# kolinko/effort

Hardware: AMD Instinct MI355X
Metric: effective GB/s + tokens/s vs effort %, Mistral-7B FFN 4096x11008 fp16 (higher is better)
Workload: dtype f16

## Files before the change

effort_amd/_lib.py:

```python
from __future__ import annotations

import ctypes as C
import os
import subprocess

_HERE = os.path.dirname(os.path.abspath(__file__))
LAB_LIB_PATH = os.path.join(_HERE, "libeffort_hip_lab.so")
LIB_PATH = (LAB_LIB_PATH if os.environ.get("EFFORT_HIP_LIB") == "lab" else os.environ.get("EFFORT_HIP_LIB")) or os.path.join(_HERE, "libeffort_hip.so")

ERRORS = {
    -1: "EFFORT_ERR_ARG", -2: "EFFORT_ERR_SHAPE", -3: "EFFORT_ERR_EFFORT", -4: "EFFORT_ERR_HIP",
    -5: "EFFORT_ERR_KIND", -6: "EFFORT_ERR_CONVERT", -7: "EFFORT_ERR_BLAS", -8: "EFFORT_ERR_COMM",
}


class EffortError(RuntimeError):
    def __init__(self, code: int, where: str, detail: str = ""):
        self.code = code
        super().__init__(f"{where}: {ERRORS.get(code, code)} {detail}".strip())


def build(verbose: bool = False) -> str:
    cmd = ["make", "-C", os.path.join(_HERE, "csrc"), "-j8", "all"]
    res = subprocess.run(cmd, capture_output=not verbose, text=True)
    if res.returncode != 0:
        raise RuntimeError("building libeffort_hip.so failed:\n" + (res.stdout or "") + (res.stderr or ""))
    return LIB_PATH


_P = C.c_void_p
_SIGS = {
    "effort_create": (_P, [C.c_int, _P]),
    "effort_destroy": (None, [_P]),
    "effort_set_stream": (C.c_int, [_P, _P]),
    "effort_sync": (C.c_int, [_P]),
    "effort_set_overlap": (C.c_int, [_P, C.c_int]),
    "effort_set_row_reuse": (C.c_int, [_P, C.c_int]),
    "effort_join": (C.c_int, [_P]),
    "effort_last_error": (C.c_char_p, [_P]),
    "effort_version": (C.c_char_p, []),
    "effort_weights_fp16": (_P, [_P, _P, _P, _P, C.c_int, C.c_int, C.c_int, C.c_int]),
    "effort_weights_fp16_pitched": (_P, [_P, _P, C.c_int, _P, _P, C.c_int, C.c_int, C.c_int, C.c_int]),
    "effort_aligned_row_pitch": (C.c_int, [C.c_int]),
    "effort_weights_q4": (_P, [_P, _P, _P, _P, _P, C.c_int64, C.c_int, C.c_int, C.c_int]),
    "effort_weights_free": (None, [_P]),
    "effort_weights_refresh": (C.c_int, [_P]),
    "effort_weights_align_rows": (C.c_int, [_P]),
    "effort_weights_row_pitch": (C.c_int, [_P]),
    "effort_weights_get_bound": (C.c_int, [_P, C.POINTER(C.c_float)]),
    "effort_weights_set_bound": (C.c_int, [_P, C.POINTER(C.c_float)]),
    "effort_weights_column_shard": (_P, [_P, C.c_int, C.c_int]),
    "effort_comm_unique_id": (C.c_int, [_P]),
    "effort_comm_create": (C.c_int, [_P, C.c_int, C.c_int, _P]),
    "effort_comm_destroy": (C.c_int, [_P]),
    "effort_comm_rank": (C.c_int, [_P]),
    "effort_comm_world": (C.c_int, [_P]),
    "effort_allgather_outputs": (C.c_int, [_P, _P, _P, C.c_int]),
    "effort_bucketmul": (C.c_int, [_P, _P, _P, _P, _P, C.c_double]),
    "effort_bucketmul_q4": (C.c_int, [_P, _P, _P, _P, _P, C.c_double]),
    "effort_bucketmul_group": (C.c_int, [_P, C.c_int, _P, _P, _P, _P, _P]),
    "effort_bucketmul_q4_group": (C.c_int, [_P, C.c_int, _P, _P, _P, _P, _P]),
    "effort_bucketmul_group_fused": (C.c_int, [_P, C.c_int, _P, _P, _P, _P, _P, _P, _P, _P]),
    "effort_bucketmul_q4_group_fused": (C.c_int, [_P, C.c_int, _P, _P, _P, _P, _P, _P, _P, _P]),
    "effort_group_dispatch_count": (C.c_int, [_P, C.c_int, C.POINTER(C.c_uint32)]),
    "effort_group_cutoff": (C.c_int, [_P, C.c_int, C.POINTER(C.c_float)]),
    "effort_debug_occupancy": (C.c_int, [_P, C.c_int, C.c_int, C.c_int, C.c_int]),
    "effort_set_persistent": (C.c_int, [_P, C.c_int]),
    "effort_debug_hook_lane": (C.c_int, [_P, C.c_int]),
    "effort_add_rmsnorm_mul": (C.c_int, [_P, _P, _P, _P, _P, C.c_int]),
    "effort_rope_kv": (C.c_int, [_P, _P, _P, _P, _P, _P, _P, _P, C.c_int, C.c_int, C.c_int, C.c_int, C.c_float]),
    "effort_attention": (C.c_int, [_P, _P, _P, _P, _P, _P, C.c_int, C.c_int, C.c_int]),
    "effort_rope_attention": (C.c_int, [_P, _P, _P, _P, _P, _P, _P, _P, C.c_int, C.c_int, C.c_int, C.c_int, C.c_float]),
    "effort_silu_mul": (C.c_int, [_P, _P, _P, _P, C.c_int]),
    "effort_fetch_row": (C.c_int, [_P, _P, _P, _P, C.c_int]),
    "effort_argmax": (C.c_int, [_P, _P, C.c_int, _P, _P, _P, C.c_int]),
    "effort_decode_status": (C.c_int, [_P, C.POINTER(C.c_int)]),
    "effort_sample": (C.c_int, [_P, _P, C.c_int, _P, _P, _P, _P, C.c_int, _P, _P]),
    "effort_topk": (C.c_int, [_P, _P, C.c_int, C.c_int, _P, _P]),
    "effort_sample_bits": (C.c_uint32, [C.c_uint32, C.c_uint32, C.c_uint32, C.c_uint32]),
    "effort_convert_status": (C.c_int, [_P, C.POINTER(C.c_int)]),
    "effort_q4_outlier_count": (C.c_int64, [C.c_int, C.c_int, C.c_double]),
    "effort_convert_q4": (C.c_int, [_P, _P, C.c_int, C.c_int, C.c_double, _P, _P, _P, _P]),
    "effort_top2_softmax": (C.c_int, [_P, _P, C.c_int, _P, _P]),
    "effort_mix2": (C.c_int, [_P, _P, _P, _P, _P, C.c_int]),
    "effort_moe_route": (C.c_int, [_P, _P, _P, _P, C.c_int, C.c_int, _P, _P, _P]),
    "effort_mix2_add": (C.c_int, [_P, _P, _P, _P, _P, C.c_int]),
    "effort_dense_gemv": (C.c_int, [_P, _P, _P, _P, C.c_int, C.c_int]),
    "effort_dense_gemv_expert": (C.c_int, [_P, _P, _P, _P, _P, C.c_int, C.c_int, C.c_int]),
    "effort_dense_gemm_rows": (C.c_int, [_P, _P, _P, _P, C.c_int, C.c_int, C.c_int]),
    "effort_dense_gemm_rows_routed": (C.c_int, [_P, _P, C.c_int, _P, _P, C.c_int, _P, C.c_int, C.c_int, C.c_int]),
    "effort_weights_bucket_dense_ok": (C.c_int, [_P, C.POINTER(C.c_int)]),
    "effort_bucket_gemm_rows": (C.c_int, [_P, _P, C.c_int, _P, _P, C.c_int]),
    "effort_bucket_gemm_rows_routed": (C.c_int, [_P, _P, _P, _P, C.c_int, _P, C.c_int]),
    "effort_moe_route_rows": (C.c_int, [_P, _P, _P, _P, C.c_int, C.c_int, _P, _P, _P, C.c_int]),
    "effort_mix2_add_rows": (C.c_int, [_P, _P, _P, _P, C.c_int, C.c_int]),
    "effort_fetch_rows": (C.c_int, [_P, _P, _P, _P, C.c_int, C.c_int]),
    "effort_add_rmsnorm_mul_rows": (C.c_int, [_P, _P, _P, _P, _P, C.c_int, C.c_int]),
    "effort_rope_kv_rows": (C.c_int, [_P, _P, _P, _P, _P, _P, _P, C.c_int, C.c_int, C.c_int, C.c_int, C.c_int, C.c_int, C.c_float]),
    "effort_attention_rows": (C.c_int, [_P, _P, _P, _P, C.c_int, C.c_int, _P, C.c_int, C.c_int, C.c_int]),
    "effort_attention_block": (C.c_int, [_P, _P, _P, _P, C.c_int, C.c_int, _P, C.c_int, C.c_int, C.c_int]),
    "effort_set_dense_backend": (C.c_int, [_P, C.c_int]),
    "effort_last_dispatch_count": (C.c_int, [_P, C.POINTER(C.c_uint32)]),
    "effort_last_cutoff": (C.c_int, [_P, C.POINTER(C.c_float)]),
    "effort_calc_dispatch": (C.c_int, [_P, _P, _P, _P, C.c_double, _P, _P]),
    "effort_convert_fp16": (C.c_int, [_P, _P, C.c_int, C.c_int, _P, _P, _P]),
    "effort_convert_fp16_pitched": (C.c_int, [_P, _P, C.c_int, C.c_int, _P, C.c_int, _P, _P]),
    "effort_cosine": (C.c_int, [_P, _P, _P, C.c_int, C.POINTER(C.c_float)]),
    "effort_set_split_cutoff": (C.c_int, [_P, C.c_int]),
    "effort_set_tuning": (C.c_int, [_P, C.c_int, C.c_int, C.c_int]),
    "effort_is_lab_build": (C.c_int, []),
    "effort_enable_kernel_timing": (C.c_int, [_P, C.c_int]),
    "effort_debug_stamps": (C.c_int, [_P, C.POINTER(C.c_ulonglong)]),
    "effort_debug_slice_counts": (C.c_int, [_P, C.c_int, C.POINTER(C.c_uint32), C.c_int]),
    "effort_debug_plan": (C.c_int, [C.c_int, C.c_int, C.c_int, C.c_int, _P, _P, _P, _P, _P, _P, C.c_int, C.c_int, C.c_int, C.c_int, _P, _P, _P, _P, _P, _P, _P, _P, _P]),
    "effort_debug_check_bundle": (C.c_int, [C.c_int, C.c_int, C.c_int, C.c_int, C.c_int, C.c_int]),
    "effort_debug_variants": (C.c_int, [C.c_int, _P, C.c_int]),
    "effort_debug_last_variant": (C.c_int, [_P, C.c_int, _P]),
    "effort_debug_lanes": (C.c_int, [C.c_int, C.c_int, _P, C.c_int64, _P]),
    "effort_debug_trace": (C.c_int, [_P, C.POINTER(C.c_ulonglong), C.c_int]),
    "effort_kernel_clock": (C.c_int, [_P, C.POINTER(C.c_double), C.POINTER(C.c_int)]),
    "effort_kernel_timing": (C.c_int, [_P, C.POINTER(C.c_double), C.POINTER(C.c_double), C.POINTER(C.c_double), C.POINTER(C.c_int)]),
}

_lib = None


def lib() -> C.CDLL:
    global _lib
    if _lib is None:
        if not os.path.exists(LIB_PATH):
            raise RuntimeError(
                f"{LIB_PATH} is missing: the HIP extension has not been built "
                "(run `python -c 'import __graft_entry__ as g; g.build()'` or `make -C effort_amd/csrc`). "
                "effort_amd has no CPU fallback.")
        import torch
        l = C.CDLL(LIB_PATH)
        for name, (res, args) in _SIGS.items():
            if (name.startswith("effort_debug_") or name == "effort_is_lab_build") and os.environ.get("EFFORT_HIP_LIB") and not hasattr(l, name):
                continue
            fn = getattr(l, name)
            fn.restype = res
            fn.argtypes = args
        _lib = l
    return _lib


def exported_symbols() -> list[str]:
    return sorted(_SIGS)
```

effort_amd/csrc/glue.hip:

```cpp
#include <rocblas/rocblas.h>

#include "host.h"
#include "prefill.h"
#include "sample_device.h"

using namespace effort;

extern "C" int effort_set_dense_backend(effort_ctx* c, int rocblas) {
    if (!c) return EFFORT_ERR_ARG;
    c->denseRocblas = rocblas != 0;
    return EFFORT_OK;
}
void dense_release(effort_ctx* c) { if (c->blas) rocblas_destroy_handle(c->blas); c->blas = nullptr; }
void dense_set_stream(effort_ctx* c) { if (c->blas) rocblas_set_stream(c->blas, c->stream); }
extern "C" int effort_dense_gemv(effort_ctx* c, const void* W, const float* v, float* out, int inDim, int outDim) {
    if (!c || !W || !v || !out || inDim <= 0 || outDim <= 0) return fail(c, EFFORT_ERR_ARG, "dense_gemv: bad argument");
    JOIN_TRY(c);
    if (inDim % 16) return fail(c, EFFORT_ERR_SHAPE, "dense_gemv: inDim % 16 != 0 (helpers/mps.swift:18)");
    if (!c->denseRocblas && dense_gemv_supported((uint32_t)inDim, (uint32_t)outDim)) {
        HIP_TRY(c, launch_dense_gemv(static_cast<const uint16_t*>(W), v, out, (uint32_t)inDim, (uint32_t)outDim, c->stream));
        return EFFORT_OK;
    }
    if (!c->blas) {
        if (rocblas_create_handle(&c->blas) != rocblas_status_success) return fail(c, EFFORT_ERR_BLAS, "rocblas_create_handle");
        rocblas_set_stream(c->blas, c->stream);
        rocblas_set_pointer_mode(c->blas, rocblas_pointer_mode_host);
    }
    OK_TRY(c->d_vhalf.grow(c, (size_t)inDim, (size_t)inDim));
    HIP_TRY(c, launch_f32_to_f16(v, c->d_vhalf.buf, inDim, c->stream));
    const float alpha = 1.0f, beta = 0.0f;
    rocblas_status s = rocblas_hssgemv_strided_batched(c->blas, rocblas_operation_transpose, inDim, outDim, &alpha,
                                                       static_cast<const rocblas_half*>(W), inDim, 0,
                                                       reinterpret_cast<const rocblas_half*>(c->d_vhalf.buf), 1, 0, &beta, out, 1, 0, 1);
    if (s != rocblas_status_success) return fail(c, EFFORT_ERR_BLAS, "rocblas_hssgemv_strided_batched");
    return EFFORT_OK;
}
extern "C" int effort_dense_gemv_expert(effort_ctx* c, const void* W, const uint32_t* expNo, const float* v, float* out, int inDim, int outDim,
                                        int numExperts) {
    if (!c || !W || !expNo || !v || !out || inDim <= 0 || outDim <= 0 || numExperts <= 0) return fail(c, EFFORT_ERR_ARG, "dense_gemv_expert: bad argument");
    JOIN_TRY(c);
    if (!dense_gemv_supported((uint32_t)inDim, (uint32_t)outDim) || (size_t)numExperts * outDim * inDim * 2 > 0xFFFFFFFFull)
        return fail(c, EFFORT_ERR_SHAPE, "dense_gemv_expert: inDim % 16 != 0, inDim > 65536, or a stack of 4 GiB or more");
    return HIP_RC(c, launch_dense_gemv_expert(static_cast<const uint16_t*>(W), expNo, v, out, (uint32_t)inDim, (uint32_t)outDim, (uint32_t)numExperts, c->stream));
}

extern "C" int effort_convert_fp16_pitched(effort_ctx* c, const void* W, int outDim, int inDim, void* buckets, int rowPitchBytes, void* stats, void* probes) {
    if (!c || !W || !buckets || !stats || !probes) return fail(c, EFFORT_ERR_ARG, "convert_fp16: null argument");
    JOIN_TRY(c);
    if (outDim <= 0 || inDim < kProbes || !(outDim >= kProbes || kProbes % outDim == 0) || outDim > 16384 || inDim > 32000 ||
        outDim % 16 || (outDim / 16) % 4)
        return fail(c, EFFORT_ERR_CONVERT, "convert_fp16: bucketize preconditions violated");
    const int pitch = rowPitchBytes ? rowPitchBytes : outDim / 16 * 2;
    if (pitch < outDim / 16 * 2 || pitch % 8) return fail(c, EFFORT_ERR_CONVERT, "convert_fp16: row pitch must be a multiple of 8 bytes >= 2*cols");
    const size_t elems = (size_t)outDim * inDim;
    OK_TRY(c->d_convVals.grow(c, elems, elems));
    return HIP_RC(c, launch_convert_fp16(static_cast<const uint16_t*>(W), outDim, inDim, static_cast<uint16_t*>(buckets), (uint32_t)pitch / 2u,
                                   static_cast<uint16_t*>(stats), static_cast<uint16_t*>(probes), c->d_convVals.buf, c->d_status, c->stream));
}
extern "C" int effort_convert_fp16(effort_ctx* c, const void* W, int outDim, int inDim, void* buckets, void* stats, void* probes) {
    return effort_convert_fp16_pitched(c, W, outDim, inDim, buckets, 0, stats, probes);
}

extern "C" int64_t effort_q4_outlier_count(int inDim, int outDim, double perc) {
    if (inDim <= 0 || outDim <= 0 || !(perc >= 0.0 && perc <= 1.0)) return EFFORT_ERR_ARG;
    return (int64_t)((double)((int64_t)inDim * outDim) * perc);
}
extern "C" int effort_convert_q4(effort_ctx* c, const void* core2, int inDim, int outDim, double perc, void* buckets, void* stats, void* probes,
                                 void* outliers) {
    if (!c || !core2 || !buckets || !stats || !probes) return fail(c, EFFORT_ERR_ARG, "convert_q4: null argument");
    JOIN_TRY(c);
    if (inDim <= 0 || outDim <= 0 || outDim % 32 || (int64_t)inDim * outDim >= (1ll << 32) || !(perc >= 0.0 && perc <= 1.0))
        return fail(c, EFFORT_ERR_CONVERT, "convert_q4: outDim % 32 != 0 (q4_draft.py:299), or a matrix of 2^32 elements or more");
    const int64_t cnt = effort_q4_outlier_count(inDim, outDim, perc);
    if (cnt >= (1ll << 31)) return fail(c, EFFORT_ERR_CONVERT, "convert_q4: 2^31 outliers or more (the candidate sort counts in int)");
    if (cnt > 0 && !outliers) return fail(c, EFFORT_ERR_ARG, "convert_q4: outliers buffer missing");
    hipSetDevice(c->device);
    return HIP_RC(c, launch_convert_q4(static_cast<const uint16_t*>(core2), (uint32_t)inDim, (uint32_t)outDim, (uint32_t)cnt, static_cast<uint16_t*>(buckets),
                                 static_cast<float*>(stats), static_cast<uint16_t*>(probes), static_cast<float*>(outliers), c->env.numCU, c->stream));
}

extern "C" int effort_cosine(effort_ctx* c, const float* a, const float* b, int n, float* host_out) {
    if (!c || !a || !b || !host_out || n <= 0) return EFFORT_ERR_ARG;
    JOIN_TRY(c);
    HIP_TRY(c, launch_cosine(a, b, n, c->d_cos, c->stream));
    HIP_TRY(c, hipMemcpyAsync(host_out, c->d_cos, 4, hipMemcpyDeviceToHost, c->stream));
    return HIP_RC(c, hipStreamSynchronize(c->stream));
}

extern "C" int effort_add_rmsnorm_mul(effort_ctx* c, float* h, const float* delta, const void* w, float* out, int n) {
    if (!c || !h || !w || !out || n <= 0) return fail(c, EFFORT_ERR_ARG, "add_rmsnorm_mul: bad argument");
    JOIN_TRY(c);
    return HIP_RC(c, launch_add_rmsnorm_mul(h, delta, static_cast<const uint16_t*>(w), out, (uint32_t)n, c->stream));
}
extern "C" int effort_rope_kv(effort_ctx* c, const float* xq, const float* xk, const float* xv, float* qOut, float* kCache,
                              float* vCache, const uint32_t* pos, int numHeads, int numHeadsKV, int headDim, int maxTokens, float ropeBase) {
    if (!c || !xq || !xk || !xv || !qOut || !kCache || !vCache || !pos) return fail(c, EFFORT_ERR_ARG, "rope_kv: null argument");
    JOIN_TRY(c);
    if (numHeads <= 0 || numHeadsKV <= 0 || numHeads % numHeadsKV || headDim < 2 || headDim > 1024 || headDim % 2 || !(ropeBase > 1.0f) || maxTokens <= 0)
        return fail(c, EFFORT_ERR_SHAPE, "rope_kv: bad head geometry");
    return HIP_RC(c, launch_rope_kv(xq, xk, xv, qOut, kCache, vCache, pos, numHeads, numHeadsKV, headDim, ropeBase, (uint32_t)maxTokens, c->d_status + 1, c->stream));
}
extern "C" int effort_attention(effort_ctx* c, const float* q, const float* kCache, const float* vCache, const uint32_t* pos,
                                float* out, int numHeads, int headDim, int maxTokens) {
    if (!c || !q || !kCache || !vCache || !pos || !out) return fail(c, EFFORT_ERR_ARG, "attention: null argument");
    JOIN_TRY(c);
    if (numHeads <= 0 || maxTokens <= 0 || maxTokens > 8192 || (headDim != 64 && headDim != 128 && headDim != 256))
        return fail(c, EFFORT_ERR_SHAPE, "attention: headDim 64/128/256, maxTokens <= 8192");
    return HIP_RC(c, launch_attention(q, kCache, vCache, pos, out, numHeads, headDim, maxTokens, c->stream));
}
extern "C" int effort_rope_attention(effort_ctx* c, const float* xq, const float* xk, const float* xv, float* kCache, float* vCache,
                                     const uint32_t* pos, float* out, int numHeads, int numHeadsKV, int headDim, int maxTokens, float ropeBase) {
    if (!c || !xq || !xk || !xv || !kCache || !vCache || !pos || !out) return fail(c, EFFORT_ERR_ARG, "rope_attention: null argument");
    JOIN_TRY(c);
    if (numHeads <= 0 || numHeadsKV <= 0 || numHeads % numHeadsKV || maxTokens <= 0 || maxTokens > 8192 || !(ropeBase > 1.0f) ||
        (headDim != 64 && headDim != 128 && headDim != 256))
        return fail(c, EFFORT_ERR_SHAPE, "rope_attention: headDim 64/128/256, maxTokens <= 8192");
    return HIP_RC(c, launch_rope_attention(xq, xk, xv, kCache, vCache, pos, out, numHeads, numHeadsKV, headDim, maxTokens, ropeBase, c->d_status + 1, c->stream));
}
extern "C" int effort_silu_mul(effort_ctx* c, const float* x1, const float* x3, float* out, int n) {
    if (!c || !x1 || !x3 || !out || n <= 0) return fail(c, EFFORT_ERR_ARG, "silu_mul: bad argument");
    JOIN_TRY(c);
    return HIP_RC(c, launch_silu_mul(x1, x3, out, (uint32_t)n, c->stream));
}
extern "C" int effort_fetch_row(effort_ctx* c, const void* emb, const uint32_t* id, float* out, int n) {
    if (!c || !emb || !id || !out || n <= 0) return fail(c, EFFORT_ERR_ARG, "fetch_row: bad argument");
    JOIN_TRY(c);
    return HIP_RC(c, launch_fetch_row(static_cast<const uint16_t*>(emb), id, out, (uint32_t)n, c->stream));
}
static_assert(EFFORT_PREFILL_MAX_ROWS == 64, "prefill.hip: kPrefillMaxRows, four token tiles of 16");
static bool prefill_rows_ok(int rows) { return rows >= 1 && rows <= EFFORT_PREFILL_MAX_ROWS; }
extern "C" int effort_dense_gemm_rows(effort_ctx* c, const void* W, const float* x, float* out, int inDim, int outDim, int rows) {
    if (inDim <= 0 || outDim <= 0 || !prefill_rows_ok(rows)) return fail(c, EFFORT_ERR_ARG, "dense_gemm_rows: inDim, outDim >= 1, 1 <= rows <= 64");
    if (!dense_gemm_rows_supported((uint32_t)inDim, (uint32_t)outDim))
        return fail(c, EFFORT_ERR_SHAPE, "dense_gemm_rows: inDim % 32 == 0, inDim <= 65536, outDim <= 2^24, W below 4 GiB");
    if (!c || !W || !x || !out) return fail(c, EFFORT_ERR_ARG, "dense_gemm_rows: null argument");
    JOIN_TRY(c);
    OK_TRY(c->d_xhRows.grow(c, (size_t)rows * inDim, (size_t)EFFORT_PREFILL_MAX_ROWS * inDim));
    OK_TRY(c->d_gemmPart.grow(c, dense_gemm_rows_partial_floats((uint32_t)inDim, (uint32_t)outDim, (uint32_t)rows),
                              dense_gemm_rows_partial_floats((uint32_t)inDim, (uint32_t)outDim, EFFORT_PREFILL_MAX_ROWS)));
    return HIP_RC(c, launch_dense_gemm_rows(static_cast<const uint16_t*>(W), x, c->d_xhRows.buf, c->d_gemmPart.buf, out, (uint32_t)inDim, (uint32_t)outDim,
                                      (uint32_t)rows, c->stream));
}
extern "C" int effort_dense_gemm_rows_routed(effort_ctx* c, const void* W, int numExperts, const uint32_t* idx2, const float* x, int xPerSlot, float* out,
                                             int inDim, int outDim, int rows) {
    if (inDim <= 0 || outDim <= 0 || numExperts <= 0 || !prefill_rows_ok(rows) || (xPerSlot != 0 && xPerSlot != 1))
        return fail(c, EFFORT_ERR_ARG, "dense_gemm_rows_routed: inDim, outDim, numExperts >= 1, 1 <= rows <= 64, xPerSlot 0 / 1");
    if (!dense_gemm_rows_supported((uint32_t)inDim, (uint32_t)outDim) || numExperts > 64)
        return fail(c, EFFORT_ERR_SHAPE, "dense_gemm_rows_routed: inDim % 32 == 0, inDim <= 65536, outDim <= 2^24, one expert below 4 GiB, numExperts <= 64");
    if (!c || !W || !idx2 || !x || !out) return fail(c, EFFORT_ERR_ARG, "dense_gemm_rows_routed: null argument");
    JOIN_TRY(c);
    const size_t xRows = (size_t)(xPerSlot ? 2 : 1) * rows;
    OK_TRY(c->d_xhRouted.grow(c, xRows * inDim, (size_t)2 * EFFORT_PREFILL_MAX_ROWS * inDim));
    OK_TRY(c->d_routedPart.grow(c, dense_gemm_rows_routed_partial_floats((uint32_t)inDim, (uint32_t)outDim, (uint32_t)rows),
                                dense_gemm_rows_routed_partial_floats((uint32_t)inDim, (uint32_t)outDim, EFFORT_PREFILL_MAX_ROWS)));
    OK_TRY(c->d_routedGroups.grow(c, dense_gemm_rows_routed_group_words(), dense_gemm_rows_routed_group_words()));
    return HIP_RC(c, launch_dense_gemm_rows_routed(static_cast<const uint16_t*>(W), (uint32_t)numExperts, idx2, x, (uint32_t)xPerSlot, c->d_xhRouted.buf,
                                             c->d_routedPart.buf, c->d_routedGroups.buf, out, (uint32_t)inDim, (uint32_t)outDim, (uint32_t)rows, c->stream));
}
static int bucket_handle_shape(const effort_w* w, const char* name) {
    char what[128];
    if (w->fmt != kFp16) { snprintf(what, sizeof(what), "%s: an FP16 bundle (Q4 buckets hold no whole matrix)", name); return fail(w->ctx, EFFORT_ERR_KIND, what); }
    if (w->rowsPerIn != 16u || w->view || w->inDim % 32u || !bucket_gemm_rows_supported(w->inDim, w->outDim)) {
        snprintf(what, sizeof(what), "%s: percentLoad 16, a full handle (no column shard), inDim %% 32 == 0", name);
        return fail(w->ctx, EFFORT_ERR_SHAPE, what);
    }
    return EFFORT_OK;
}
static int bucket_dense_state(const effort_w* w, int* ok) {
    effort_ctx* c = w->ctx;
    if (w->bucketDense < 0) {
        int bad = 0;
        hipSetDevice(c->device);
        JOIN_TRY(c);
        HIP_TRY(c, hipMemsetAsync(c->d_status + 2, 0, 4, c->stream));
        HIP_TRY(c, launch_bucket_dense_check(w->buckets, w->rowPitch, w->cols, w->inDim, w->numExperts, c->d_status + 2, c->stream));
        HIP_TRY(c, hipMemcpyAsync(&bad, c->d_status + 2, 4, hipMemcpyDeviceToHost, c->stream));
        HIP_TRY(c, hipStreamSynchronize(c->stream));
        w->bucketDense = bad ? 0 : 1;
    }
    *ok = w->bucketDense;
    return EFFORT_OK;
}
extern "C" int effort_weights_bucket_dense_ok(effort_w* w, int* host_out) {
    if (!w || !w->ctx || w->dead || !host_out) return EFFORT_ERR_ARG;
    OK_TRY(bucket_handle_shape(w, "weights_bucket_dense_ok"));
    return bucket_dense_state(w, host_out);
}
static int bucket_refuse_collisions(effort_ctx* c, const effort_w* w, const char* name) {
    int ok = 0;
    OK_TRY(bucket_dense_state(w, &ok));
    if (ok) return EFFORT_OK;
    char what[160];
    snprintf(what, sizeof(what), "%s: the bundle is not un-bucketable (two entries of one bucket name the same output: effort_convert_status reported drops)", name);
    return fail(c, EFFORT_ERR_CONVERT, what);
}
extern "C" int effort_bucket_gemm_rows(effort_ctx* c, const effort_w* w, int expert, const float* x, float* out, int rows) {
    if (!w || w->dead) return fail(c, EFFORT_ERR_ARG, "bucket_gemm_rows: null handle");
    if (!prefill_rows_ok(rows) || expert < 0 || (uint32_t)expert >= w->numExperts) return fail(c, EFFORT_ERR_ARG, "bucket_gemm_rows: 1 <= rows <= 64, 0 <= expert < numExperts");
    OK_TRY(bucket_handle_shape(w, "bucket_gemm_rows"));
    if (!c || c != w->ctx || !x || !out) return fail(c, EFFORT_ERR_ARG, "bucket_gemm_rows: null argument (or a handle of another context)");
    JOIN_TRY(c);
    OK_TRY(bucket_refuse_collisions(c, w, "bucket_gemm_rows"));
    OK_TRY(c->d_xhRows.grow(c, (size_t)rows * w->inDim, (size_t)EFFORT_PREFILL_MAX_ROWS * w->inDim));
    OK_TRY(c->d_gemmPart.grow(c, dense_gemm_rows_partial_floats(w->inDim, w->outDim, (uint32_t)rows),
                              dense_gemm_rows_partial_floats(w->inDim, w->outDim, EFFORT_PREFILL_MAX_ROWS)));
    const uint16_t* B = reinterpret_cast<const uint16_t*>(reinterpret_cast<const unsigned char*>(w->buckets) + (size_t)expert * 16u * w->inDim * w->rowPitch);
    return HIP_RC(c, launch_bucket_gemm_rows(B, w->rowPitch, x, c->d_xhRows.buf, c->d_gemmPart.buf, out, w->inDim, w->outDim, (uint32_t)rows, c->stream));
}
extern "C" int effort_bucket_gemm_rows_routed(effort_ctx* c, const effort_w* w, const uint32_t* idx2, const float* x, int xPerSlot, float* out, int rows) {
    if (!w || w->dead) return fail(c, EFFORT_ERR_ARG, "bucket_gemm_rows_routed: null handle");
    if (!prefill_rows_ok(rows) || (xPerSlot != 0 && xPerSlot != 1)) return fail(c, EFFORT_ERR_ARG, "bucket_gemm_rows_routed: 1 <= rows <= 64, xPerSlot 0 / 1");
    OK_TRY(bucket_handle_shape(w, "bucket_gemm_rows_routed"));
    if (w->numExperts > 64u) return fail(c, EFFORT_ERR_SHAPE, "bucket_gemm_rows_routed: numExperts <= 64");
    if (!c || c != w->ctx || !idx2 || !x || !out) return fail(c, EFFORT_ERR_ARG, "bucket_gemm_rows_routed: null argument (or a handle of another context)");
    JOIN_TRY(c);
    OK_TRY(bucket_refuse_collisions(c, w, "bucket_gemm_rows_routed"));
    const size_t xRows = (size_t)(xPerSlot ? 2 : 1) * rows;
    OK_TRY(c->d_xhRouted.grow(c, xRows * w->inDim, (size_t)2 * EFFORT_PREFILL_MAX_ROWS * w->inDim));
    OK_TRY(c->d_routedPart.grow(c, dense_gemm_rows_routed_partial_floats(w->inDim, w->outDim, (uint32_t)rows),
                                dense_gemm_rows_routed_partial_floats(w->inDim, w->outDim, EFFORT_PREFILL_MAX_ROWS)));
    OK_TRY(c->d_routedGroups.grow(c, dense_gemm_rows_routed_group_words(), dense_gemm_rows_routed_group_words()));
    return HIP_RC(c, launch_bucket_gemm_rows_routed(w->buckets, w->rowPitch, w->numExperts, idx2, x, (uint32_t)xPerSlot, c->d_xhRouted.buf, c->d_routedPart.buf,
                                              c->d_routedGroups.buf, out, w->inDim, w->outDim, (uint32_t)rows, c->stream));
}
extern "C" int effort_moe_route_rows(effort_ctx* c, const float* h, const void* normW, const void* gateW, int n, int numExperts, float* gateOut,
                                     uint32_t* idx2, float* val2, int rows) {
    if (n <= 0 || numExperts <= 0 || !prefill_rows_ok(rows)) return fail(c, EFFORT_ERR_ARG, "moe_route_rows: n, numExperts >= 1, 1 <= rows <= 64");
    if (!moe_route_supported((uint32_t)n, (uint32_t)numExperts))
        return fail(c, EFFORT_ERR_SHAPE, "moe_route_rows: n % 16 == 0, 16 <= n <= 16384, 1 <= numExperts <= 64");
    if (!c || !h || !normW || !gateW || !idx2 || !val2) return fail(c, EFFORT_ERR_ARG, "moe_route_rows: null argument");
    JOIN_TRY(c);
    return HIP_RC(c, launch_moe_route_rows(h, static_cast<const uint16_t*>(normW), static_cast<const uint16_t*>(gateW), (uint32_t)n, (uint32_t)numExperts, gateOut,
                                     idx2, val2, (uint32_t)rows, c->stream));
}
extern "C" int effort_mix2_add_rows(effort_ctx* c, float* h, const float* f, const float* val2, int n, int rows) {
    if (n <= 0 || !prefill_rows_ok(rows)) return fail(c, EFFORT_ERR_ARG, "mix2_add_rows: n >= 1, 1 <= rows <= 64");
    if (!c || !h || !f || !val2) return fail(c, EFFORT_ERR_ARG, "mix2_add_rows: null argument");
    JOIN_TRY(c);
    return HIP_RC(c, launch_mix2_add_rows(h, f, val2, (uint32_t)n, (uint32_t)rows, c->stream));
}
extern "C" int effort_fetch_rows(effort_ctx* c, const void* emb, const uint32_t* ids, float* out, int n, int rows) {
    if (n <= 0 || !prefill_rows_ok(rows)) return fail(c, EFFORT_ERR_ARG, "fetch_rows: n >= 1, 1 <= rows <= 64");
    if (!c || !emb || !ids || !out) return fail(c, EFFORT_ERR_ARG, "fetch_rows: null argument");
    JOIN_TRY(c);
    return HIP_RC(c, launch_fetch_rows(static_cast<const uint16_t*>(emb), ids, out, (uint32_t)n, (uint32_t)rows, c->stream));
}
extern "C" int effort_add_rmsnorm_mul_rows(effort_ctx* c, float* h, const float* delta, const void* w, float* out, int n, int rows) {
    if (n <= 0 || !prefill_rows_ok(rows)) return fail(c, EFFORT_ERR_ARG, "add_rmsnorm_mul_rows: n >= 1, 1 <= rows <= 64");
    if (!c || !h || !w || !out) return fail(c, EFFORT_ERR_ARG, "add_rmsnorm_mul_rows: null argument");
    JOIN_TRY(c);
    return HIP_RC(c, launch_add_rmsnorm_mul_rows(h, delta, static_cast<const uint16_t*>(w), out, (uint32_t)n, (uint32_t)rows, c->stream));
}
static bool prefill_range_ok(int pos0, int rows, int maxTokens) {
    return prefill_rows_ok(rows) && pos0 >= 0 && maxTokens > 0 && pos0 <= maxTokens - rows;
}
extern "C" int effort_rope_kv_rows(effort_ctx* c, const float* xq, const float* xk, const float* xv, float* qOut, float* kCache, float* vCache,
                                   int pos0, int rows, int numHeads, int numHeadsKV, int headDim, int maxTokens, float ropeBase) {
    if (!prefill_range_ok(pos0, rows, maxTokens)) return fail(c, EFFORT_ERR_ARG, "rope_kv_rows: 1 <= rows <= 64, 0 <= pos0, pos0 + rows <= maxTokens");
    if (numHeads <= 0 || numHeadsKV <= 0 || numHeads % numHeadsKV || headDim < 2 || headDim > 1024 || headDim % 2 || !(ropeBase > 1.0f))
        return fail(c, EFFORT_ERR_SHAPE, "rope_kv_rows: bad head geometry");
    if (!c || !xq || !xk || !xv || !qOut || !kCache || !vCache) return fail(c, EFFORT_ERR_ARG, "rope_kv_rows: null argument");
    JOIN_TRY(c);
    return HIP_RC(c, launch_rope_kv_rows(xq, xk, xv, qOut, kCache, vCache, (uint32_t)pos0, (uint32_t)rows, numHeads, numHeadsKV, headDim, ropeBase, c->stream));
}
static int prefill_attention(effort_ctx* c, const char* name, decltype(&launch_attention_rows) launch, const float* q, const float* kCache,
                             const float* vCache, int pos0, int rows, float* out, int numHeads, int headDim, int maxTokens) {
    char what[96];
    auto refuse = [&](int code, const char* why) { snprintf(what, sizeof(what), "%s: %s", name, why); return fail(c, code, what); };
    if (!prefill_range_ok(pos0, rows, maxTokens)) return refuse(EFFORT_ERR_ARG, "1 <= rows <= 64, 0 <= pos0, pos0 + rows <= maxTokens");
    if (numHeads <= 0 || maxTokens > 8192 || (headDim != 64 && headDim != 128 && headDim != 256))
        return refuse(EFFORT_ERR_SHAPE, "headDim 64/128/256, maxTokens <= 8192");
    if (!c || !q || !kCache || !vCache || !out) return refuse(EFFORT_ERR_ARG, "null argument");
    JOIN_TRY(c);
    return hip_rc(c, name, launch(q, kCache, vCache, (uint32_t)pos0, (uint32_t)rows, out, numHeads, headDim, c->stream));
}
extern "C" int effort_attention_rows(effort_ctx* c, const float* q, const float* kCache, const float* vCache, int pos0, int rows, float* out,
                                     int numHeads, int headDim, int maxTokens) {
    return prefill_attention(c, "attention_rows", launch_attention_rows, q, kCache, vCache, pos0, rows, out, numHeads, headDim, maxTokens);
}
extern "C" int effort_attention_block(effort_ctx* c, const float* q, const float* kCache, const float* vCache, int pos0, int rows, float* out,
                                      int numHeads, int headDim, int maxTokens) {
    return prefill_attention(c, "attention_block", launch_attention_block, q, kCache, vCache, pos0, rows, out, numHeads, headDim, maxTokens);
}
extern "C" int effort_top2_softmax(effort_ctx* c, const float* gate, int n, uint32_t* idx2, float* val2) {
    if (!c || !gate || !idx2 || !val2 || n < 1) return fail(c, EFFORT_ERR_ARG, "top2_softmax: bad argument");
    JOIN_TRY(c);
    return HIP_RC(c, launch_top2_softmax(gate, (uint32_t)n, idx2, val2, c->stream));
}
extern "C" int effort_mix2(effort_ctx* c, const float* f0, const float* f1, const float* val2, float* out, int n) {
    if (!c || !f0 || !f1 || !val2 || !out || n <= 0) return fail(c, EFFORT_ERR_ARG, "mix2: bad argument");
    JOIN_TRY(c);
    return HIP_RC(c, launch_mix2(f0, f1, val2, out, (uint32_t)n, c->stream));
}
extern "C" int effort_moe_route(effort_ctx* c, const float* h, const void* normW, const void* gateW, int n, int numExperts, float* gateOut,
                                uint32_t* idx2, float* val2) {
    if (!c || !h || !normW || !gateW || !idx2 || !val2) return fail(c, EFFORT_ERR_ARG, "moe_route: null argument");
    JOIN_TRY(c);
    if (n <= 0 || numExperts <= 0 || !moe_route_supported((uint32_t)n, (uint32_t)numExperts))
        return fail(c, EFFORT_ERR_SHAPE, "moe_route: n % 16 == 0, 16 <= n <= 16384, 1 <= numExperts <= 64");
    return HIP_RC(c, launch_moe_route(h, static_cast<const uint16_t*>(normW), static_cast<const uint16_t*>(gateW), (uint32_t)n, (uint32_t)numExperts, gateOut,
                                idx2, val2, c->stream));
}
extern "C" int effort_mix2_add(effort_ctx* c, float* h, const float* f0, const float* f1, const float* val2, int n) {
    if (!c || !h || !f0 || !f1 || !val2 || n <= 0) return fail(c, EFFORT_ERR_ARG, "mix2_add: bad argument");
    JOIN_TRY(c);
    return HIP_RC(c, launch_mix2_add(h, f0, f1, val2, (uint32_t)n, c->stream));
}
extern "C" int effort_argmax(effort_ctx* c, const float* logits, int n, uint32_t* idOut, uint32_t* pos, uint32_t* history, int historyLen) {
    if (!c || !logits || !idOut || !pos || n <= 0 || (history && historyLen <= 0)) return fail(c, EFFORT_ERR_ARG, "argmax: bad argument");
    JOIN_TRY(c);
    return HIP_RC(c, launch_argmax(logits, (uint32_t)n, idOut, pos, history, (uint32_t)(history ? historyLen : 0), c->d_status + 1, c->stream));
}
extern "C" int effort_sample(effort_ctx* c, const float* logits, int n, const effort_sample_params* params, uint32_t* idOut, uint32_t* pos,
                             uint32_t* history, int historyLen, uint32_t* topkIdx, float* topkVal) {
    if (!c || !logits || !params || !idOut || !pos || n <= 0 || (history && historyLen <= 0)) return fail(c, EFFORT_ERR_ARG, "sample: bad argument");
    JOIN_TRY(c);
    return HIP_RC(c, launch_sample(logits, (uint32_t)n, params, idOut, pos, history, (uint32_t)(history ? historyLen : 0), c->d_status + 1, topkIdx, topkVal,
                             c->stream));
}
extern "C" int effort_topk(effort_ctx* c, const float* logits, int n, int k, uint32_t* idx, float* val) {
    if (!c || !logits || !idx || !val || n <= 0 || k < 1 || k > EFFORT_SAMPLE_MAX_K) return fail(c, EFFORT_ERR_ARG, "topk: bad argument (1 <= k <= 64)");
    JOIN_TRY(c);
    return HIP_RC(c, launch_topk(logits, (uint32_t)n, (uint32_t)k, idx, val, c->stream));
}
extern "C" uint32_t effort_sample_bits(uint32_t seedLo, uint32_t seedHi, uint32_t stream, uint32_t pos) { return philox_x0(seedLo, seedHi, stream, pos); }

static int read_and_clear(effort_ctx* c, int* word, int* host_out) {
    if (!c || !host_out) return EFFORT_ERR_ARG;
    JOIN_TRY(c);
    HIP_TRY(c, hipMemcpyAsync(host_out, word, 4, hipMemcpyDeviceToHost, c->stream));
    HIP_TRY(c, hipMemsetAsync(word, 0, 4, c->stream));
    return HIP_RC(c, hipStreamSynchronize(c->stream));
}
extern "C" int effort_decode_status(effort_ctx* c, int* host_out) { return read_and_clear(c, c ? c->d_status + 1 : nullptr, host_out); }
extern "C" int effort_convert_status(effort_ctx* c, int* host_out) { return read_and_clear(c, c ? c->d_status : nullptr, host_out); }
```

effort_amd/csrc/host.h:

```cpp
#pragma once
#include <cstdio>
#include <cstring>
#include <new>

#include "../../include/effort_hip.h"
#include "../../include/effort_hip_debug.h"
#include "effort_internal.h"
#include "lanes.h"
#include "plan.h"

struct ncclComm;
struct _rocblas_handle;

struct Lane {
    hipStream_t own = nullptr;
    hipEvent_t done = nullptr;
    bool dirty = false;
    float* d_cutoff = nullptr;
    uint32_t* d_count = nullptr;
    float* d_slabs = nullptr;
    uint32_t* d_counters = nullptr;
    uint32_t* d_sliceCounts = nullptr;
    uint32_t* d_queue = nullptr;
    uint32_t lastCalls = 1, lastSliceOff[effort::kMaxGroup] = {0}, lastSlices[effort::kMaxGroup] = {0};
    uint32_t lastLaunches = 0;
    effort::LaunchedVariant lastVariant[effort::kMaxLaunches] = {};
};

template <typename T>
struct Scratch {
    T* buf = nullptr;
    size_t have = 0;
    int grow(effort_ctx* c, size_t need, size_t want);
    void release() { hipFree(buf); buf = nullptr; have = 0; }
};
#define EFFORT_CTX_SCRATCH(X)                                                                                                              \
    X(uint16_t, d_vhalf)                                                                         \
    X(uint16_t, d_xhRows)        \
    X(float, d_gemmPart)                                                           \
    X(uint16_t, d_xhRouted)      \
    X(float, d_routedPart) X(uint32_t, d_routedGroups)          \
    X(uint16_t, d_convVals)

struct effort_ctx {
    static constexpr uint32_t kMaxTiles = 1024, kMaxSlices = 4096;
    static constexpr size_t kSlabBytes = (size_t)64 << 20;
    int device = 0;
    hipStream_t stream = nullptr;
    effort::PlanEnv env = scratch_env();
    static effort::PlanEnv scratch_env() { effort::PlanEnv e; e.slabBytes = kSlabBytes; e.maxTiles = kMaxTiles; e.maxSlices = kMaxSlices; return e; }
    Lane lane[effort::kMaxLanes];
    effort::LaneBook book;
    int lastLane = 0;
    hipEvent_t forkEv = nullptr;
    uint32_t* d_blockScratch = nullptr;
#define EFFORT_X(T, name) Scratch<T> name;
    EFFORT_CTX_SCRATCH(EFFORT_X)
#undef EFFORT_X
    float* d_cos = nullptr;
    int* d_status = nullptr;
    unsigned long long* d_tstamp = nullptr;
    double wallClockKHz = 100000.0;
    _rocblas_handle* blas = nullptr;
    ncclComm* comm = nullptr;
    int commRank = 0, commWorld = 1;
    bool denseRocblas = false;
    bool rowReuse = false;
    bool timing = false;
    bool trace = false;
    static constexpr int kMaxSamples = 4096;
    hipEvent_t* ev = nullptr;
    int nSamples = 0;
    char err[256] = {0};
};

struct effort_w {
    effort_ctx* ctx = nullptr;
    effort::Format fmt = effort::kFp16;
    const uint16_t* buckets = nullptr;
    const uint16_t* bucketsSrc = nullptr;
    uint16_t* aligned = nullptr;
    uint32_t rowPitch = 0;
    uint32_t srcPitch = 0;
    const void* stats = nullptr;
    const uint16_t* probes = nullptr;
    uint32_t inDim = 0, outDim = 0, rowsPerIn = 0, numExperts = 1, cols = 0;
    bool view = false;
    effort_w* parent = nullptr;
    uint32_t viewTrim = 0;
    int views = 0;
    bool dead = false;
    float* rankBound = nullptr;
    uint16_t* means16 = nullptr;
    mutable int bucketDense = -1;
    uint64_t nOutliers = 0;
    uint32_t* olBlockPtr = nullptr;
    uint32_t* olEntry = nullptr;
    uint32_t* olMeta = nullptr;
};

static inline int fail(effort_ctx* c, int code, const char* what, hipError_t e = hipSuccess) {
    if (c) {
        if (e != hipSuccess) snprintf(c->err, sizeof(c->err), "%s: %s", what, hipGetErrorString(e));
        else snprintf(c->err, sizeof(c->err), "%s", what);
    }
    return code;
}
static inline int hip_rc(effort_ctx* c, const char* what, hipError_t e) { return e == hipSuccess ? EFFORT_OK : fail(c, EFFORT_ERR_HIP, what, e); }
#define HIP_RC(ctx, call) hip_rc((ctx), #call, (call))
#define OK_TRY(step) do { const int rc_ = (step); if (rc_ != EFFORT_OK) return rc_; } while (0)
#define HIP_TRY(ctx, call) OK_TRY(HIP_RC(ctx, call))
#define JOIN_TRY(ctx) OK_TRY(join_lanes(ctx))

template <typename T>
int Scratch<T>::grow(effort_ctx* c, size_t need, size_t want) {
    if (need <= have) return EFFORT_OK;
    HIP_TRY(c, hipStreamSynchronize(c->stream));
    release();
    HIP_TRY(c, hipMalloc(&buf, want * sizeof(T)));
    have = want;
    return EFFORT_OK;
}

int join_lanes(effort_ctx* c);
struct LaneChoice {
    bool laned = false;
    effort::LanePick pick;
    effort::LaunchRanges ranges;
    unsigned long long capNow = 0;
    bool forked = false;
};
int choose_lane(effort_ctx* c, LaneChoice& lc, int n, const effort_w* const* ws, const float* const* vs, const uint32_t* const* expNos,
                float* const* outs, const void* const* vAux, const float* const* resids);
int fork_lane(effort_ctx* c, LaneChoice& lc);
int check_shape(uint32_t inDim, uint32_t outDim);
int check_bundle(effort::Format fmt, int inDim, int outDim, int percentLoad, int numExperts, int rowPitchBytes, uint32_t* pitchOut);
void comm_release(effort_ctx* c);
void dense_release(effort_ctx* c);
void dense_set_stream(effort_ctx* c);
```

effort_amd/csrc/prefill.h:

```cpp
#pragma once
#include "effort_internal.h"

namespace effort {

constexpr int kPrefillMaxRows = 64;
constexpr uint32_t kPfStage = 256;
constexpr size_t kPfKeepBytes = 64u << 20;
constexpr uint32_t kPfMaxAssign = 2u * kPrefillMaxRows, kPfMaxExperts = 64;

typedef _Float16 pf_half8 __attribute__((ext_vector_type(8)));
typedef float pf_f32x4 __attribute__((ext_vector_type(4)));

struct PfSplit { uint32_t per, splits; };
PfSplit pf_split(uint32_t inDim, uint32_t outDim);

hipError_t launch_rows_to_f16(const float* x, uint16_t* xh, uint32_t n, hipStream_t st);
hipError_t launch_reduce_splits(const float* part, float* out, uint32_t n, uint32_t splits, hipStream_t st);
hipError_t launch_routed_prologue(const float* x, uint16_t* xh, uint32_t n, const uint32_t* idx2, uint32_t assigns, uint32_t numExperts, uint32_t* cnt,
                                  uint32_t* list, hipStream_t st);

bool bucket_gemm_rows_supported(uint32_t inDim, uint32_t outDim);
hipError_t launch_bucket_dense_check(const uint16_t* B, uint32_t pitch, uint32_t cols, uint32_t inDim, uint32_t numExperts, int* bad, hipStream_t st);
hipError_t launch_bucket_gemm_rows(const uint16_t* B, uint32_t pitch, const float* x, uint16_t* xh, float* part, float* out, uint32_t inDim,
                                   uint32_t outDim, uint32_t rows, hipStream_t st);
hipError_t launch_bucket_gemm_rows_routed(const uint16_t* B, uint32_t pitch, uint32_t numExperts, const uint32_t* idx2, const float* x, uint32_t xPerSlot,
                                          uint16_t* xh, float* part, uint32_t* groups, float* out, uint32_t inDim, uint32_t outDim, uint32_t rows,
                                          hipStream_t st);

}
```

effort_amd/csrc/prefill_buckets.hip:

```cpp
#include <type_traits>

#include "prefill.h"

namespace effort {

constexpr uint32_t kBkCols = 32;
constexpr uint32_t kBkRows = 16u * kBkCols;
constexpr uint32_t kBkWaves = 8, kBkThreads = 64u * kBkWaves;
constexpr uint32_t kBkTiles = kBkRows / 16u / kBkWaves;
constexpr uint32_t kBkK = 64;
constexpr uint32_t kBkPitch = kBkK * 2u + 16u;
constexpr uint32_t kBkTileBytes = kBkRows * kBkPitch;
constexpr uint32_t kBkLds = kBkTileBytes + 64u * kBkPitch;
static_assert(kPfStage % kBkK == 0 && kBkTileBytes % (16u * kBkThreads) == 0, "whole chunks per stage; the fill is whole 16-byte stores");

template <int NT, int AUX, int VEC, bool ROUTED>
__device__ __forceinline__ void bucket_rows_body(unsigned char* __restrict__ lds, const uint16_t* __restrict__ B, uint32_t pitch, uint32_t cols,
                                                 const uint16_t* __restrict__ xh, float* __restrict__ o, uint32_t inDim, uint32_t outDim, uint32_t live,
                                                 uint32_t xRows, uint32_t per, const uint32_t* col, uint32_t xShift) {
    constexpr uint32_t kPiecesPerRow = kBkCols * 2u / (4u * VEC);
    constexpr int kLoads = (int)(16u * kBkK * kPiecesPerRow / kBkThreads);
    constexpr uint32_t kXPieces = NT * 16u * (kBkK / 8u);
    constexpr int kXLoads = (int)((kXPieces + kBkThreads - 1u) / kBkThreads);
    unsigned char* const tile = lds;
    unsigned char* const xs = lds + kBkTileBytes;
    const uint32_t tid = threadIdx.x, lane = tid & 63u, wave = __builtin_amdgcn_readfirstlane(tid >> 6);
    const uint32_t g = lane >> 4, r16 = lane & 15u, c0 = blockIdx.x * kBkCols;
    const __amdgpu_buffer_rsrc_t rs = __builtin_amdgcn_make_buffer_rsrc(const_cast<uint16_t*>(B), 0, (int)((16u * inDim - 1u) * pitch + cols * 2u), 0x00020000);
    const __amdgpu_buffer_rsrc_t xr = __builtin_amdgcn_make_buffer_rsrc(const_cast<uint16_t*>(xh), 0, (int)(xRows * inDim * 2u), 0x00020000);
    const uint32_t chunks = (inDim + kPfStage - 1u) / kPfStage * (kPfStage / kBkK);
    const uint32_t q0 = blockIdx.y * per * (kPfStage / kBkK), q1 = min(q0 + per * (kPfStage / kBkK), chunks);

    constexpr int kDepth = VEC == 4 && !ROUTED ? 2 : 1;
    uint32_t heldA[kDepth][kLoads][VEC];
    uint4 heldX[kDepth][kXLoads];
    auto ask_a = [&](uint32_t q, uint32_t (&nextA)[kLoads][VEC]) {
#pragma unroll
        for (int i = 0; i < kLoads; i++) {
            const uint32_t idx = tid + (uint32_t)i * kBkThreads, brow = idx / kPiecesPerRow, p = idx % kPiecesPerRow;
            const uint32_t rank = brow / kBkK, j = q * kBkK + brow % kBkK, cFirst = c0 + p * 2u * VEC;
#pragma unroll
            for (int v = 0; v < VEC; v++) nextA[i][v] = 0u;
            if (j < inDim && cFirst + 2u * VEC <= cols) {
                const uint32_t off = (rank * inDim + j) * pitch + cFirst * 2u;
                if constexpr (VEC == 4) {
                    const auto w = __builtin_amdgcn_raw_buffer_load_b128(rs, off, 0, AUX);
                    nextA[i][0] = w[0]; nextA[i][1] = w[1]; nextA[i][2] = w[2]; nextA[i][3] = w[3];
                } else {
                    nextA[i][0] = __builtin_amdgcn_raw_buffer_load_b32(rs, off, 0, AUX);
                }
            }
        }
    };
    auto x_row = [&](uint32_t tok) -> uint32_t {
        if constexpr (ROUTED) return tok < live ? col[tok] >> xShift : 0u;
        else return min(tok, live - 1u);
    };
    auto ask_x = [&](uint32_t q, uint4 (&nextX)[kXLoads]) {
#pragma unroll
        for (int i = 0; i < kXLoads; i++) {
            const uint32_t idx = tid + (uint32_t)i * kBkThreads, tok = idx / (kBkK / 8u), e = q * kBkK + (idx % (kBkK / 8u)) * 8u;
            nextX[i] = make_uint4(0u, 0u, 0u, 0u);
            if (idx < kXPieces && tok < live && e < inDim) {
                const auto x = __builtin_amdgcn_raw_buffer_load_b128(xr, x_row(tok) * inDim * 2u + e * 2u, 0, 0);
                nextX[i] = make_uint4(x[0], x[1], x[2], x[3]);
            }
        }
    };
    auto scatter = [&](const uint32_t (&nextA)[kLoads][VEC], const uint4 (&nextX)[kXLoads]) {
#pragma unroll
        for (int i = 0; i < kLoads; i++) {
            const uint32_t idx = tid + (uint32_t)i * kBkThreads, brow = idx / kPiecesPerRow, p = idx % kPiecesPerRow;
            const uint32_t jj = brow % kBkK, cLocal = p * 2u * VEC;
#pragma unroll
            for (int v = 0; v < VEC; v++)
#pragma unroll
                for (int h = 0; h < 2; h++) {
                    const uint32_t w = (nextA[i][v] >> (16 * h)) & 0xFFFFu;
                    const uint32_t row = (cLocal + 2u * v + h) * 16u + (w & 15u);
                    if (w != 0u) *reinterpret_cast<uint16_t*>(tile + row * kBkPitch + jj * 2u) = (uint16_t)w;
                }
        }
#pragma unroll
        for (int i = 0; i < kXLoads; i++) {
            const uint32_t idx = tid + (uint32_t)i * kBkThreads;
            if (idx < kXPieces) *reinterpret_cast<uint4*>(xs + (idx / (kBkK / 8u)) * kBkPitch + (idx % (kBkK / 8u)) * 16u) = nextX[i];
        }
    };

    pf_f32x4 acc[kBkTiles][NT];
#pragma unroll
    for (int m = 0; m < (int)kBkTiles; m++)
#pragma unroll
        for (int t = 0; t < NT; t++) acc[m][t] = pf_f32x4{0.0f, 0.0f, 0.0f, 0.0f};
    auto chunk = [&](uint32_t q, auto slotTag) {
        constexpr int slot = decltype(slotTag)::value;
#pragma unroll
        for (int i = 0; i < (int)(kBkTileBytes / (16u * kBkThreads)); i++)
            *reinterpret_cast<uint4*>(tile + (tid + (uint32_t)i * kBkThreads) * 16u) = make_uint4(0u, 0u, 0u, 0u);
        __syncthreads();
        scatter(heldA[slot], heldX[slot]);
        __syncthreads();
        if (q + kDepth < q1) { ask_a(q + kDepth, heldA[slot]); ask_x(q + kDepth, heldX[slot]); }
        __builtin_amdgcn_sched_barrier(0);
#pragma unroll
        for (int u = 0; u < 2; u++) {
            pf_half8 bf[NT];
#pragma unroll
            for (int t = 0; t < NT; t++) bf[t] = *reinterpret_cast<const pf_half8*>(xs + (t * 16u + r16) * kBkPitch + (g * 2u + u) * 16u);
#pragma unroll
            for (int m = 0; m < (int)kBkTiles; m++) {
                const pf_half8 af = *reinterpret_cast<const pf_half8*>(tile + ((wave * kBkTiles + m) * 16u + r16) * kBkPitch + (g * 2u + u) * 16u);
#pragma unroll
                for (int t = 0; t < NT; t++) acc[m][t] = __builtin_amdgcn_mfma_f32_16x16x32_f16(af, bf[t], acc[m][t], 0, 0, 0);
            }
        }
        __builtin_amdgcn_sched_barrier(0);
        __syncthreads();
    };
    ask_a(q0, heldA[0]);
    ask_x(q0, heldX[0]);
    if constexpr (kDepth == 2) {
        if (q0 + 1u < q1) { ask_a(q0 + 1u, heldA[1]); ask_x(q0 + 1u, heldX[1]); }
        for (uint32_t q = q0; q < q1; q += 2u) {
            chunk(q, std::integral_constant<int, 0>{});
            if (q + 1u < q1) chunk(q + 1u, std::integral_constant<int, 1>{});
        }
    } else {
        for (uint32_t q = q0; q < q1; q++) chunk(q, std::integral_constant<int, 0>{});
    }
#pragma unroll
    for (int t = 0; t < NT; t++) {
        const uint32_t tok = t * 16u + r16;
        uint32_t orow = tok;
        if constexpr (ROUTED) orow = tok < live ? col[tok] : 0u;
#pragma unroll
        for (int m = 0; m < (int)kBkTiles; m++)
#pragma unroll
            for (int i = 0; i < 4; i++) {
                const uint32_t row = c0 * 16u + (wave * kBkTiles + m) * 16u + g * 4u + i;
                if (tok < live && row < outDim) o[(size_t)orow * outDim + row] = acc[m][t][i];
            }
    }
}

template <int NT, int AUX, int VEC>
__global__ __launch_bounds__(kBkThreads) void bucket_gemm_rows_kernel(const uint16_t* __restrict__ B, uint32_t pitch, uint32_t cols,
                                                                      const uint16_t* __restrict__ xh, float* __restrict__ dst, uint32_t inDim,
                                                                      uint32_t outDim, uint32_t rows, uint32_t per) {
    extern __shared__ __attribute__((aligned(16))) unsigned char bk_lds[];
    bucket_rows_body<NT, AUX, VEC, false>(bk_lds, B, pitch, cols, xh, dst + (size_t)blockIdx.y * rows * outDim, inDim, outDim, rows, rows, per, nullptr, 0u);
}

template <int AUX, int VEC>
__global__ __launch_bounds__(kBkThreads) void bucket_gemm_rows_routed_kernel(const uint16_t* __restrict__ B, uint32_t pitch, uint32_t cols,
                                                                             const uint16_t* __restrict__ xh, float* __restrict__ dst,
                                                                             const uint32_t* __restrict__ cnt, const uint32_t* __restrict__ list,
                                                                             uint32_t inDim, uint32_t outDim, uint32_t assigns, uint32_t xRows,
                                                                             uint32_t xShift, uint32_t per) {
    extern __shared__ __attribute__((aligned(16))) unsigned char bk_lds[];
    __shared__ uint32_t col[64];
    const uint32_t e = blockIdx.z, n = __builtin_amdgcn_readfirstlane(min(cnt[e], kPfMaxAssign));
    if (n == 0u) return;
    const uint16_t* Be = reinterpret_cast<const uint16_t*>(reinterpret_cast<const unsigned char*>(B) + (size_t)e * 16u * inDim * pitch);
    float* o = dst + (size_t)blockIdx.y * assigns * outDim;
    for (uint32_t a0 = 0; a0 < n; a0 += 64u) {
        const uint32_t live = min(n - a0, 64u);
        if (threadIdx.x < live) col[threadIdx.x] = min(list[e * kPfMaxAssign + a0 + threadIdx.x], assigns - 1u);
        __syncthreads();
        switch ((live + 15u) / 16u) {
            case 1: bucket_rows_body<1, AUX, VEC, true>(bk_lds, Be, pitch, cols, xh, o, inDim, outDim, live, xRows, per, col, xShift); break;
            case 2: bucket_rows_body<2, AUX, VEC, true>(bk_lds, Be, pitch, cols, xh, o, inDim, outDim, live, xRows, per, col, xShift); break;
            case 3: bucket_rows_body<3, AUX, VEC, true>(bk_lds, Be, pitch, cols, xh, o, inDim, outDim, live, xRows, per, col, xShift); break;
            default: bucket_rows_body<4, AUX, VEC, true>(bk_lds, Be, pitch, cols, xh, o, inDim, outDim, live, xRows, per, col, xShift); break;
        }
        __syncthreads();
    }
}

__global__ __launch_bounds__(256) void bucket_dense_check_kernel(const uint16_t* __restrict__ B, uint32_t pitch, uint32_t cols, uint32_t inDim, int* bad) {
    const uint32_t cp = blockIdx.x * 256u + threadIdx.x, j = blockIdx.y, e = blockIdx.z;
    if (cp >= cols / 2u) return;
    const unsigned char* base = reinterpret_cast<const unsigned char*>(B) + ((size_t)e * 16u * inDim + j) * pitch + cp * 4u;
    uint32_t seen0 = 0u, seen1 = 0u, dup = 0u;
    for (uint32_t r = 0; r < 16u; r++) {
        const uint32_t w = *reinterpret_cast<const uint32_t*>(base + (size_t)r * inDim * pitch), w0 = w & 0xFFFFu, w1 = w >> 16;
        const uint32_t b0 = w0 ? 1u << (w0 & 15u) : 0u, b1 = w1 ? 1u << (w1 & 15u) : 0u;
        dup |= (seen0 & b0) | (seen1 & b1);
        seen0 |= b0; seen1 |= b1;
    }
    if (dup) atomicOr(bad, 1);
}

bool bucket_gemm_rows_supported(uint32_t inDim, uint32_t outDim) {
    return dense_gemm_rows_supported(inDim, outDim) && outDim % 32u == 0 && outDim <= 16384u;
}

hipError_t launch_bucket_dense_check(const uint16_t* B, uint32_t pitch, uint32_t cols, uint32_t inDim, uint32_t numExperts, int* bad, hipStream_t st) {
    hipLaunchKernelGGL(bucket_dense_check_kernel, dim3((cols / 2u + 255u) / 256u, inDim, numExperts), dim3(256), 0, st, B, pitch, cols, inDim, bad);
    return hipGetLastError();
}

static bool bucket_wide(const uint16_t* B, uint32_t pitch, uint32_t cols) {
    return pitch % 16u == 0 && reinterpret_cast<uintptr_t>(B) % 16u == 0 && cols % 8u == 0;
}

template <int NT, int AUX, int VEC>
static hipError_t launch_bucket_gemm_rows_t(const uint16_t* B, uint32_t pitch, uint32_t cols, const uint16_t* xh, float* dst, uint32_t inDim,
                                            uint32_t outDim, uint32_t rows, PfSplit sp, hipStream_t st) {
    const hipError_t e = allow_full_lds(reinterpret_cast<const void*>(&bucket_gemm_rows_kernel<NT, AUX, VEC>));
    if (e != hipSuccess) return e;
    hipLaunchKernelGGL((bucket_gemm_rows_kernel<NT, AUX, VEC>), dim3((cols + kBkCols - 1u) / kBkCols, sp.splits), dim3(kBkThreads), kBkLds, st,
                       B, pitch, cols, xh, dst, inDim, outDim, rows, sp.per);
    return hipGetLastError();
}
template <int NT>
static hipError_t launch_bucket_gemm_rows_nt(bool nt, bool wide, const uint16_t* B, uint32_t pitch, uint32_t cols, const uint16_t* xh, float* dst,
                                             uint32_t inDim, uint32_t outDim, uint32_t rows, PfSplit sp, hipStream_t st) {
    if (nt) return wide ? launch_bucket_gemm_rows_t<NT, 2, 4>(B, pitch, cols, xh, dst, inDim, outDim, rows, sp, st)
                        : launch_bucket_gemm_rows_t<NT, 2, 1>(B, pitch, cols, xh, dst, inDim, outDim, rows, sp, st);
    return wide ? launch_bucket_gemm_rows_t<NT, 0, 4>(B, pitch, cols, xh, dst, inDim, outDim, rows, sp, st)
                : launch_bucket_gemm_rows_t<NT, 0, 1>(B, pitch, cols, xh, dst, inDim, outDim, rows, sp, st);
}

hipError_t launch_bucket_gemm_rows(const uint16_t* B, uint32_t pitch, const float* x, uint16_t* xh, float* part, float* out, uint32_t inDim,
                                   uint32_t outDim, uint32_t rows, hipStream_t st) {
    if (rows < 1u || rows > (uint32_t)kPrefillMaxRows) return hipErrorInvalidValue;
    hipError_t e = launch_rows_to_f16(x, xh, rows * inDim, st);
    if (e != hipSuccess) return e;
    const PfSplit sp = pf_split(inDim, outDim);
    float* dst = sp.splits > 1u ? part : out;
    const uint32_t cols = outDim / 16u;
    const bool nt = (size_t)inDim * outDim * 2u > kPfKeepBytes, wide = bucket_wide(B, pitch, cols);
    switch ((rows + 15u) / 16u) {
        case 1: e = launch_bucket_gemm_rows_nt<1>(nt, wide, B, pitch, cols, xh, dst, inDim, outDim, rows, sp, st); break;
        case 2: e = launch_bucket_gemm_rows_nt<2>(nt, wide, B, pitch, cols, xh, dst, inDim, outDim, rows, sp, st); break;
        case 3: e = launch_bucket_gemm_rows_nt<3>(nt, wide, B, pitch, cols, xh, dst, inDim, outDim, rows, sp, st); break;
        default: e = launch_bucket_gemm_rows_nt<4>(nt, wide, B, pitch, cols, xh, dst, inDim, outDim, rows, sp, st); break;
    }
    if (e != hipSuccess || sp.splits == 1u) return e;
    return launch_reduce_splits(part, out, rows * outDim, sp.splits, st);
}

template <int AUX, int VEC>
static hipError_t launch_bucket_gemm_rows_routed_t(const uint16_t* B, uint32_t pitch, uint32_t cols, uint32_t numExperts, const uint16_t* xh, float* dst,
                                                   const uint32_t* cnt, const uint32_t* list, uint32_t inDim, uint32_t outDim, uint32_t assigns,
                                                   uint32_t xRows, uint32_t xShift, PfSplit sp, hipStream_t st) {
    const hipError_t e = allow_full_lds(reinterpret_cast<const void*>(&bucket_gemm_rows_routed_kernel<AUX, VEC>));
    if (e != hipSuccess) return e;
    hipLaunchKernelGGL((bucket_gemm_rows_routed_kernel<AUX, VEC>), dim3((cols + kBkCols - 1u) / kBkCols, sp.splits, numExperts), dim3(kBkThreads), kBkLds, st,
                       B, pitch, cols, xh, dst, cnt, list, inDim, outDim, assigns, xRows, xShift, sp.per);
    return hipGetLastError();
}

hipError_t launch_bucket_gemm_rows_routed(const uint16_t* B, uint32_t pitch, uint32_t numExperts, const uint32_t* idx2, const float* x, uint32_t xPerSlot,
                                          uint16_t* xh, float* part, uint32_t* groups, float* out, uint32_t inDim, uint32_t outDim, uint32_t rows,
                                          hipStream_t st) {
    if (rows < 1u || rows > (uint32_t)kPrefillMaxRows || numExperts < 1u || numExperts > kPfMaxExperts || xPerSlot > 1u) return hipErrorInvalidValue;
    const uint32_t assigns = 2u * rows, xRows = xPerSlot ? assigns : rows, cols = outDim / 16u;
    uint32_t* cnt = groups;
    uint32_t* list = groups + kPfMaxExperts;
    hipError_t e = launch_routed_prologue(x, xh, xRows * inDim, idx2, assigns, numExperts, cnt, list, st);
    if (e != hipSuccess) return e;
    const PfSplit sp = pf_split(inDim, outDim);
    float* dst = sp.splits > 1u ? part : out;
    const uint32_t xShift = xPerSlot ? 0u : 1u;
    const bool nt = (size_t)inDim * outDim * 2u > kPfKeepBytes;
    const bool wide = bucket_wide(B, pitch, cols);
    if (nt) e = wide ? launch_bucket_gemm_rows_routed_t<2, 4>(B, pitch, cols, numExperts, xh, dst, cnt, list, inDim, outDim, assigns, xRows, xShift, sp, st)
                     : launch_bucket_gemm_rows_routed_t<2, 1>(B, pitch, cols, numExperts, xh, dst, cnt, list, inDim, outDim, assigns, xRows, xShift, sp, st);
    else e = wide ? launch_bucket_gemm_rows_routed_t<0, 4>(B, pitch, cols, numExperts, xh, dst, cnt, list, inDim, outDim, assigns, xRows, xShift, sp, st)
                  : launch_bucket_gemm_rows_routed_t<0, 1>(B, pitch, cols, numExperts, xh, dst, cnt, list, inDim, outDim, assigns, xRows, xShift, sp, st);
    if (e != hipSuccess || sp.splits == 1u) return e;
    return launch_reduce_splits(part, out, assigns * outDim, sp.splits, st);
}

}
```

include/effort_hip_debug.h:

```cpp
#ifndef EFFORT_HIP_DEBUG_H
#define EFFORT_HIP_DEBUG_H

#include "effort_hip.h"

#ifdef __cplusplus
extern "C" {
#endif

EFFORT_API int effort_set_tuning(effort_ctx* ctx, int wavesPerGroup, int elemsPerLane, int rowSlices);
EFFORT_API int effort_set_split_cutoff(effort_ctx* ctx, int split);

EFFORT_API int effort_set_persistent(effort_ctx* ctx, int wgPerCU);

EFFORT_API int effort_debug_hook_lane(effort_ctx* ctx, int lane);

EFFORT_API int effort_is_lab_build(void);
EFFORT_API int effort_enable_kernel_timing(effort_ctx* ctx, int enable);
EFFORT_API int effort_kernel_clock(effort_ctx* ctx, double* mul_us_avg, int* n_launches);
EFFORT_API int effort_kernel_timing(effort_ctx* ctx, double* mul_us_avg, double* cutoff_us_avg,
                         double* integrate_us_avg, int* n_samples);
EFFORT_API int effort_debug_occupancy(effort_ctx* ctx, int q4, int waves, int elems, int ldsBytes);
EFFORT_API int effort_debug_stamps(effort_ctx* ctx, unsigned long long* host32);
EFFORT_API int effort_debug_slice_counts(effort_ctx* ctx, int idx, uint32_t* host, int maxSlices);
EFFORT_API int effort_debug_plan(int q4, int numCU, int lanes, int n, const int* inDim, const int* outDim, const int* percentLoad,
                      const int* prologue, const int* hasResid, const double* effort, int persistent, int tuneW, int tuneE, int tuneS,
                      int* we, int* slices, int* tiles, int* sliceRows, int* launchOf,
                      int* launchPersistent, int* launchCutJobs, int* launchCompact, int* launchStagger);
EFFORT_API int effort_debug_check_bundle(int q4, int inDim, int outDim, int percentLoad, int numExperts, int rowPitchBytes);
EFFORT_API int effort_debug_variants(int q4, int* rows, int maxRows);
EFFORT_API int effort_debug_last_variant(effort_ctx* ctx, int launch, int* out8);
#define EFFORT_LANES_LAUNCH 0
#define EFFORT_LANES_TIMED 1
#define EFFORT_LANES_JOIN 2
#define EFFORT_LANES_OUT_WORDS 18
EFFORT_API int effort_debug_lanes(int lanes, int nOps, const int64_t* ops, int64_t nWords, int64_t* out);
EFFORT_API int effort_debug_trace(effort_ctx* ctx, unsigned long long* host, int maxRecords);

#ifdef __cplusplus
}
#endif
#endif
```

Measured before the change: 22220.

## Retile bucket prefill GEMM with adaptive column groups and double-buffered LDS

Reworks the bucket GEMM-rows prefill kernel. Column-group width is now a template parameter (4–32 columns) picked by a cost model over CU count, with a debug override. Each WG runs 4 waves, double-buffers LDS for small groups, uses a deeper prefetch pipeline and load widths matched to the group, and swizzles the block index across 64-column lines. The fill path becomes branchless, with zero rows stored into a dummy slot, and non-temporal load hints are dropped. The aim is better occupancy and load/compute overlap for prefill, at the cost of more template variants and a heuristic that could pick a poor group size.

```diff
diff --git a/effort_amd/_lib.py b/effort_amd/_lib.py
--- a/effort_amd/_lib.py
+++ b/effort_amd/_lib.py
@@ -116,6 +116,8 @@
     "effort_debug_check_bundle": (C.c_int, [C.c_int, C.c_int, C.c_int, C.c_int, C.c_int, C.c_int]),
     "effort_debug_variants": (C.c_int, [C.c_int, _P, C.c_int]),
     "effort_debug_last_variant": (C.c_int, [_P, C.c_int, _P]),
+    "effort_debug_bucket_group": (C.c_int, [C.c_int, C.c_int, C.c_int]),
+    "effort_debug_set_bucket_group": (C.c_int, [_P, C.c_int]),
     "effort_debug_lanes": (C.c_int, [C.c_int, C.c_int, _P, C.c_int64, _P]),
     "effort_debug_trace": (C.c_int, [_P, C.POINTER(C.c_ulonglong), C.c_int]),
     "effort_kernel_clock": (C.c_int, [_P, C.POINTER(C.c_double), C.POINTER(C.c_int)]),
diff --git a/effort_amd/csrc/glue.hip b/effort_amd/csrc/glue.hip
--- a/effort_amd/csrc/glue.hip
+++ b/effort_amd/csrc/glue.hip
@@ -205,7 +205,8 @@
     OK_TRY(c->d_gemmPart.grow(c, dense_gemm_rows_partial_floats(w->inDim, w->outDim, (uint32_t)rows),
                               dense_gemm_rows_partial_floats(w->inDim, w->outDim, EFFORT_PREFILL_MAX_ROWS)));
     const uint16_t* B = reinterpret_cast<const uint16_t*>(reinterpret_cast<const unsigned char*>(w->buckets) + (size_t)expert * 16u * w->inDim * w->rowPitch);
-    return HIP_RC(c, launch_bucket_gemm_rows(B, w->rowPitch, x, c->d_xhRows.buf, c->d_gemmPart.buf, out, w->inDim, w->outDim, (uint32_t)rows, c->stream));
+    return HIP_RC(c, launch_bucket_gemm_rows(B, w->rowPitch, x, c->d_xhRows.buf, c->d_gemmPart.buf, out, w->inDim, w->outDim, (uint32_t)rows,
+                                             (uint32_t)c->env.numCU, c->bucketGroup, c->stream));
 }
 extern "C" int effort_bucket_gemm_rows_routed(effort_ctx* c, const effort_w* w, const uint32_t* idx2, const float* x, int xPerSlot, float* out, int rows) {
     if (!w || w->dead) return fail(c, EFFORT_ERR_ARG, "bucket_gemm_rows_routed: null handle");
@@ -221,7 +222,18 @@
                                 dense_gemm_rows_routed_partial_floats(w->inDim, w->outDim, EFFORT_PREFILL_MAX_ROWS)));
     OK_TRY(c->d_routedGroups.grow(c, dense_gemm_rows_routed_group_words(), dense_gemm_rows_routed_group_words()));
     return HIP_RC(c, launch_bucket_gemm_rows_routed(w->buckets, w->rowPitch, w->numExperts, idx2, x, (uint32_t)xPerSlot, c->d_xhRouted.buf, c->d_routedPart.buf,
-                                              c->d_routedGroups.buf, out, w->inDim, w->outDim, (uint32_t)rows, c->stream));
+                                              c->d_routedGroups.buf, out, w->inDim, w->outDim, (uint32_t)rows, (uint32_t)c->env.numCU, c->bucketGroup,
+                                              c->stream));
+}
+extern "C" int effort_debug_set_bucket_group(effort_ctx* c, int cols) {
+    if (!c || (cols != 0 && !bucket_group_ok((uint32_t)cols))) return EFFORT_ERR_ARG;
+    c->bucketGroup = (uint32_t)cols;
+    return EFFORT_OK;
+}
+extern "C" int effort_debug_bucket_group(int inDim, int outDim, int numCU) {
+    if (inDim <= 0 || outDim <= 0 || numCU < 1) return EFFORT_ERR_ARG;
+    if (inDim % 32 || !bucket_gemm_rows_supported((uint32_t)inDim, (uint32_t)outDim)) return EFFORT_ERR_SHAPE;
+    return (int)bucket_group_cols((uint32_t)inDim, (uint32_t)outDim, (uint32_t)numCU);
 }
 extern "C" int effort_moe_route_rows(effort_ctx* c, const float* h, const void* normW, const void* gateW, int n, int numExperts, float* gateOut,
                                      uint32_t* idx2, float* val2, int rows) {
diff --git a/effort_amd/csrc/host.h b/effort_amd/csrc/host.h
--- a/effort_amd/csrc/host.h
+++ b/effort_amd/csrc/host.h
@@ -66,6 +66,7 @@
     int commRank = 0, commWorld = 1;
     bool denseRocblas = false;
     bool rowReuse = false;
+    uint32_t bucketGroup = 0;
     bool timing = false;
     bool trace = false;
     static constexpr int kMaxSamples = 4096;
diff --git a/effort_amd/csrc/prefill.h b/effort_amd/csrc/prefill.h
--- a/effort_amd/csrc/prefill.h
+++ b/effort_amd/csrc/prefill.h
@@ -20,11 +20,13 @@
                                   uint32_t* list, hipStream_t st);
 
 bool bucket_gemm_rows_supported(uint32_t inDim, uint32_t outDim);
+uint32_t bucket_group_cols(uint32_t inDim, uint32_t outDim, uint32_t numCU);
+bool bucket_group_ok(uint32_t G);
 hipError_t launch_bucket_dense_check(const uint16_t* B, uint32_t pitch, uint32_t cols, uint32_t inDim, uint32_t numExperts, int* bad, hipStream_t st);
 hipError_t launch_bucket_gemm_rows(const uint16_t* B, uint32_t pitch, const float* x, uint16_t* xh, float* part, float* out, uint32_t inDim,
-                                   uint32_t outDim, uint32_t rows, hipStream_t st);
+                                   uint32_t outDim, uint32_t rows, uint32_t numCU, uint32_t pinG, hipStream_t st);
 hipError_t launch_bucket_gemm_rows_routed(const uint16_t* B, uint32_t pitch, uint32_t numExperts, const uint32_t* idx2, const float* x, uint32_t xPerSlot,
                                           uint16_t* xh, float* part, uint32_t* groups, float* out, uint32_t inDim, uint32_t outDim, uint32_t rows,
-                                          hipStream_t st);
+                                          uint32_t numCU, uint32_t pinG, hipStream_t st);
 
 }
diff --git a/effort_amd/csrc/prefill_buckets.hip b/effort_amd/csrc/prefill_buckets.hip
--- a/effort_amd/csrc/prefill_buckets.hip
+++ b/effort_amd/csrc/prefill_buckets.hip
@@ -4,51 +4,77 @@
 
 namespace effort {
 
-constexpr uint32_t kBkCols = 32;
-constexpr uint32_t kBkRows = 16u * kBkCols;
-constexpr uint32_t kBkWaves = 8, kBkThreads = 64u * kBkWaves;
-constexpr uint32_t kBkTiles = kBkRows / 16u / kBkWaves;
+constexpr uint32_t kBkWaves = 4, kBkThreads = 64u * kBkWaves;
 constexpr uint32_t kBkK = 64;
 constexpr uint32_t kBkPitch = kBkK * 2u + 16u;
-constexpr uint32_t kBkTileBytes = kBkRows * kBkPitch;
-constexpr uint32_t kBkLds = kBkTileBytes + 64u * kBkPitch;
-static_assert(kPfStage % kBkK == 0 && kBkTileBytes % (16u * kBkThreads) == 0, "whole chunks per stage; the fill is whole 16-byte stores");
-
-template <int NT, int AUX, int VEC, bool ROUTED>
+constexpr uint32_t kBkXBytes = 64u * kBkPitch;
+constexpr uint32_t kBkLine = 64;
+constexpr uint32_t bk_bufs(int G) { return G <= 16 ? 2u : 1u; }
+constexpr uint32_t bk_lds(int G) { return bk_bufs(G) * (16u * G * kBkPitch + kBkXBytes); }
+constexpr int bk_depth(int G, bool routed) { return routed ? (G <= 8 ? 2 : 1) : G == 4 ? 4 : G == 8 ? 3 : G == 16 ? 2 : 1; }
+static_assert(kPfStage % kBkK == 0 && kBkK == 16u * kBkWaves, "whole chunks per stage; a wave fills 16 k of every chunk");
+
+typedef uint32_t bk_u32x4 __attribute__((ext_vector_type(4), may_alias));
+typedef uint16_t bk_u16 __attribute__((may_alias));
+
+template <int I, int N, class F>
+__device__ __forceinline__ bool bk_static_while(F&& f) {
+    if constexpr (I < N) return f(std::integral_constant<int, I>{}) && bk_static_while<I + 1, N>(f);
+    else return true;
+}
+
+template <int G>
+__device__ __forceinline__ bool bk_locate(uint32_t cols, uint32_t splits, uint32_t& c0, uint32_t& split) {
+    constexpr uint32_t kPerLine = kBkLine / G;
+    const uint32_t s = blockIdx.x >> 3, k = s / kPerLine * 8u + (blockIdx.x & 7u);
+    c0 = k / splits * kBkLine + s % kPerLine * G;
+    split = k % splits;
+    return c0 < cols;
+}
+static uint32_t bk_grid(uint32_t G, uint32_t cols, uint32_t splits) {
+    const uint32_t clusters = (cols + kBkLine - 1u) / kBkLine * splits;
+    return (clusters + 7u) / 8u * 8u * (kBkLine / G);
+}
+
+template <int G, int NT, int LB, bool ROUTED>
 __device__ __forceinline__ void bucket_rows_body(unsigned char* __restrict__ lds, const uint16_t* __restrict__ B, uint32_t pitch, uint32_t cols,
                                                  const uint16_t* __restrict__ xh, float* __restrict__ o, uint32_t inDim, uint32_t outDim, uint32_t live,
-                                                 uint32_t xRows, uint32_t per, const uint32_t* col, uint32_t xShift) {
-    constexpr uint32_t kPiecesPerRow = kBkCols * 2u / (4u * VEC);
-    constexpr int kLoads = (int)(16u * kBkK * kPiecesPerRow / kBkThreads);
+                                                 uint32_t xRows, uint32_t per, const uint32_t* col, uint32_t xShift, uint32_t c0, uint32_t split) {
+    constexpr uint32_t kTileBytes = 16u * G * kBkPitch, kBufBytes = kTileBytes + kBkXBytes, kBufs = bk_bufs(G);
+    constexpr int kTiles = G / (int)kBkWaves;
+    constexpr uint32_t kPieces = 2u * G / LB, kDw = LB / 4u;
+    constexpr int kLoads = (int)(16u * 16u * kPieces / 64u);
     constexpr uint32_t kXPieces = NT * 16u * (kBkK / 8u);
     constexpr int kXLoads = (int)((kXPieces + kBkThreads - 1u) / kBkThreads);
-    unsigned char* const tile = lds;
-    unsigned char* const xs = lds + kBkTileBytes;
+    constexpr int kDepth = bk_depth(G, ROUTED);
+    static_assert(LB == 4 || LB == (2 * G < 16 ? 2 * G : 16), "a piece is dwords, or one load of up to 16 bytes");
     const uint32_t tid = threadIdx.x, lane = tid & 63u, wave = __builtin_amdgcn_readfirstlane(tid >> 6);
-    const uint32_t g = lane >> 4, r16 = lane & 15u, c0 = blockIdx.x * kBkCols;
+    const uint32_t g = lane >> 4, r16 = lane & 15u;
     const __amdgpu_buffer_rsrc_t rs = __builtin_amdgcn_make_buffer_rsrc(const_cast<uint16_t*>(B), 0, (int)((16u * inDim - 1u) * pitch + cols * 2u), 0x00020000);
     const __amdgpu_buffer_rsrc_t xr = __builtin_amdgcn_make_buffer_rsrc(const_cast<uint16_t*>(xh), 0, (int)(xRows * inDim * 2u), 0x00020000);
     const uint32_t chunks = (inDim + kPfStage - 1u) / kPfStage * (kPfStage / kBkK);
-    const uint32_t q0 = blockIdx.y * per * (kPfStage / kBkK), q1 = min(q0 + per * (kPfStage / kBkK), chunks);
-
-    constexpr int kDepth = VEC == 4 && !ROUTED ? 2 : 1;
-    uint32_t heldA[kDepth][kLoads][VEC];
+    const uint32_t q0 = split * per * (kPfStage / kBkK), q1 = min(q0 + per * (kPfStage / kBkK), chunks);
+
+    uint32_t heldA[kDepth][kLoads][kDw];
     uint4 heldX[kDepth][kXLoads];
-    auto ask_a = [&](uint32_t q, uint32_t (&nextA)[kLoads][VEC]) {
+    struct Piece { bool in; uint32_t off, jj, cLocal; };
+    auto piece = [&](uint32_t q, int i) -> Piece {
+        const uint32_t idx = lane + (uint32_t)i * 64u, p = idx % kPieces, brow = idx / kPieces;
+        const uint32_t rank = brow / 16u, jj = wave * 16u + brow % 16u, j = q * kBkK + jj, cFirst = c0 + p * (LB / 2u);
+        return Piece{j < inDim && cFirst + LB / 2u <= cols, (rank * inDim + min(j, inDim - 1u)) * pitch + min(cFirst, cols - LB / 2u) * 2u, jj, p * (LB / 2u)};
+    };
+    auto ask_a = [&](uint32_t q, uint32_t (&nextA)[kLoads][kDw]) {
 #pragma unroll
         for (int i = 0; i < kLoads; i++) {
-            const uint32_t idx = tid + (uint32_t)i * kBkThreads, brow = idx / kPiecesPerRow, p = idx % kPiecesPerRow;
-            const uint32_t rank = brow / kBkK, j = q * kBkK + brow % kBkK, cFirst = c0 + p * 2u * VEC;
-#pragma unroll
-            for (int v = 0; v < VEC; v++) nextA[i][v] = 0u;
-            if (j < inDim && cFirst + 2u * VEC <= cols) {
-                const uint32_t off = (rank * inDim + j) * pitch + cFirst * 2u;
-                if constexpr (VEC == 4) {
-                    const auto w = __builtin_amdgcn_raw_buffer_load_b128(rs, off, 0, AUX);
-                    nextA[i][0] = w[0]; nextA[i][1] = w[1]; nextA[i][2] = w[2]; nextA[i][3] = w[3];
-                } else {
-                    nextA[i][0] = __builtin_amdgcn_raw_buffer_load_b32(rs, off, 0, AUX);
-                }
+            const uint32_t off = q < q1 ? piece(q, i).off : 0u;
+            if constexpr (LB == 16) {
+                const auto w = __builtin_amdgcn_raw_buffer_load_b128(rs, off, 0, 0);
+                nextA[i][0] = w[0]; nextA[i][1] = w[1]; nextA[i][2] = w[2]; nextA[i][3] = w[3];
+            } else if constexpr (LB == 8) {
+                const auto w = __builtin_amdgcn_raw_buffer_load_b64(rs, off, 0, 0);
+                nextA[i][0] = w[0]; nextA[i][1] = w[1];
+            } else {
+                nextA[i][0] = __builtin_amdgcn_raw_buffer_load_b32(rs, off, 0, 0);
             }
         }
     };
@@ -60,119 +86,143 @@
 #pragma unroll
         for (int i = 0; i < kXLoads; i++) {
             const uint32_t idx = tid + (uint32_t)i * kBkThreads, tok = idx / (kBkK / 8u), e = q * kBkK + (idx % (kBkK / 8u)) * 8u;
-            nextX[i] = make_uint4(0u, 0u, 0u, 0u);
-            if (idx < kXPieces && tok < live && e < inDim) {
-                const auto x = __builtin_amdgcn_raw_buffer_load_b128(xr, x_row(tok) * inDim * 2u + e * 2u, 0, 0);
-                nextX[i] = make_uint4(x[0], x[1], x[2], x[3]);
-            }
-        }
-    };
-    auto scatter = [&](const uint32_t (&nextA)[kLoads][VEC], const uint4 (&nextX)[kXLoads]) {
+            const auto x = __builtin_amdgcn_raw_buffer_load_b128(xr, x_row(tok) * inDim * 2u + min(e, inDim - 8u) * 2u, 0, 0);
+            nextX[i] = make_uint4(x[0], x[1], x[2], x[3]);
+        }
+    };
+    auto fill = [&](uint32_t q, uint32_t buf, const uint32_t (&nextA)[kLoads][kDw], const uint4 (&nextX)[kXLoads]) {
+        unsigned char* const tile = lds + buf * kBufBytes;
+        unsigned char* const xs = tile + kTileBytes;
+#pragma unroll
+        for (int i = 0; i < G / 2; i++) {
+            const uint32_t idx = lane + (uint32_t)i * 64u;
+            *reinterpret_cast<bk_u32x4*>(tile + (idx / 2u) * kBkPitch + wave * 32u + (idx % 2u) * 16u) = bk_u32x4{0u, 0u, 0u, 0u};
+        }
 #pragma unroll
         for (int i = 0; i < kLoads; i++) {
-            const uint32_t idx = tid + (uint32_t)i * kBkThreads, brow = idx / kPiecesPerRow, p = idx % kPiecesPerRow;
-            const uint32_t jj = brow % kBkK, cLocal = p * 2u * VEC;
-#pragma unroll
-            for (int v = 0; v < VEC; v++)
+            const Piece pc = piece(q, i);
+#pragma unroll
+            for (int v = 0; v < (int)kDw; v++)
 #pragma unroll
                 for (int h = 0; h < 2; h++) {
-                    const uint32_t w = (nextA[i][v] >> (16 * h)) & 0xFFFFu;
-                    const uint32_t row = (cLocal + 2u * v + h) * 16u + (w & 15u);
-                    if (w != 0u) *reinterpret_cast<uint16_t*>(tile + row * kBkPitch + jj * 2u) = (uint16_t)w;
+                    const uint32_t w = pc.in ? (nextA[i][v] >> (16 * h)) & 0xFFFFu : 0u;
+                    const uint32_t row = (pc.cLocal + 2u * v + h) * 16u + (w & 15u);
+                    *reinterpret_cast<bk_u16*>(tile + row * kBkPitch + (w != 0u ? pc.jj * 2u : kBkK * 2u + (pc.jj & 7u) * 2u)) = (uint16_t)w;
                 }
         }
 #pragma unroll
         for (int i = 0; i < kXLoads; i++) {
-            const uint32_t idx = tid + (uint32_t)i * kBkThreads;
-            if (idx < kXPieces) *reinterpret_cast<uint4*>(xs + (idx / (kBkK / 8u)) * kBkPitch + (idx % (kBkK / 8u)) * 16u) = nextX[i];
-        }
-    };
-
-    pf_f32x4 acc[kBkTiles][NT];
-#pragma unroll
-    for (int m = 0; m < (int)kBkTiles; m++)
+            const uint32_t idx = tid + (uint32_t)i * kBkThreads, tok = idx / (kBkK / 8u), e = q * kBkK + (idx % (kBkK / 8u)) * 8u;
+            const uint32_t m = (tok < live && e < inDim) ? 0xFFFFFFFFu : 0u;
+            if (idx < kXPieces) *reinterpret_cast<bk_u32x4*>(xs + tok * kBkPitch + (idx % (kBkK / 8u)) * 16u) =
+                                    bk_u32x4{nextX[i].x & m, nextX[i].y & m, nextX[i].z & m, nextX[i].w & m};
+        }
+    };
+
+    pf_f32x4 acc[kTiles][NT];
+#pragma unroll
+    for (int m = 0; m < kTiles; m++)
 #pragma unroll
         for (int t = 0; t < NT; t++) acc[m][t] = pf_f32x4{0.0f, 0.0f, 0.0f, 0.0f};
-    auto chunk = [&](uint32_t q, auto slotTag) {
-        constexpr int slot = decltype(slotTag)::value;
-#pragma unroll
-        for (int i = 0; i < (int)(kBkTileBytes / (16u * kBkThreads)); i++)
-            *reinterpret_cast<uint4*>(tile + (tid + (uint32_t)i * kBkThreads) * 16u) = make_uint4(0u, 0u, 0u, 0u);
-        __syncthreads();
-        scatter(heldA[slot], heldX[slot]);
-        __syncthreads();
-        if (q + kDepth < q1) { ask_a(q + kDepth, heldA[slot]); ask_x(q + kDepth, heldX[slot]); }
-        __builtin_amdgcn_sched_barrier(0);
+    auto multiply = [&](uint32_t buf) {
+        const unsigned char* const tile = lds + buf * kBufBytes;
+        const unsigned char* const xs = tile + kTileBytes;
 #pragma unroll
         for (int u = 0; u < 2; u++) {
             pf_half8 bf[NT];
 #pragma unroll
             for (int t = 0; t < NT; t++) bf[t] = *reinterpret_cast<const pf_half8*>(xs + (t * 16u + r16) * kBkPitch + (g * 2u + u) * 16u);
 #pragma unroll
-            for (int m = 0; m < (int)kBkTiles; m++) {
-                const pf_half8 af = *reinterpret_cast<const pf_half8*>(tile + ((wave * kBkTiles + m) * 16u + r16) * kBkPitch + (g * 2u + u) * 16u);
+            for (int m = 0; m < kTiles; m++) {
+                const pf_half8 af = *reinterpret_cast<const pf_half8*>(tile + ((wave * kTiles + m) * 16u + r16) * kBkPitch + (g * 2u + u) * 16u);
 #pragma unroll
                 for (int t = 0; t < NT; t++) acc[m][t] = __builtin_amdgcn_mfma_f32_16x16x32_f16(af, bf[t], acc[m][t], 0, 0, 0);
             }
         }
+    };
+    auto refill = [&](uint32_t q, uint32_t buf, auto slotTag) {
+        constexpr int slot = decltype(slotTag)::value;
+        fill(q, buf, heldA[slot], heldX[slot]);
+        ask_a(q + kDepth, heldA[slot]);
+        ask_x(q + kDepth, heldX[slot]);
         __builtin_amdgcn_sched_barrier(0);
-        __syncthreads();
-    };
-    ask_a(q0, heldA[0]);
-    ask_x(q0, heldX[0]);
-    if constexpr (kDepth == 2) {
-        if (q0 + 1u < q1) { ask_a(q0 + 1u, heldA[1]); ask_x(q0 + 1u, heldX[1]); }
-        for (uint32_t q = q0; q < q1; q += 2u) {
-            chunk(q, std::integral_constant<int, 0>{});
-            if (q + 1u < q1) chunk(q + 1u, std::integral_constant<int, 1>{});
-        }
-    } else {
-        for (uint32_t q = q0; q < q1; q++) chunk(q, std::integral_constant<int, 0>{});
-    }
+    };
+    bk_static_while<0, kDepth>([&](auto d) {
+        constexpr uint32_t dd = decltype(d)::value;
+        ask_a(q0 + dd, heldA[dd]);
+        ask_x(q0 + dd, heldX[dd]);
+        return true;
+    });
+    refill(q0, 0u, std::integral_constant<int, 0>{});
+    __syncthreads();
+    uint32_t buf = 0u;
+    for (uint32_t q = q0;; q += kDepth)
+        if (!bk_static_while<0, kDepth>([&](auto d) {
+                constexpr int dd = decltype(d)::value;
+                const uint32_t qq = q + dd;
+                const bool more = qq + 1u < q1;
+                const std::integral_constant<int, (dd + 1) % kDepth> next{};
+                if constexpr (kBufs == 2u) refill(qq + 1u, buf ^ 1u, next);
+                multiply(buf);
+                __builtin_amdgcn_sched_barrier(0);
+                __syncthreads();
+                if constexpr (kBufs == 2u) {
+                    buf ^= 1u;
+                } else if (more) {
+                    refill(qq + 1u, 0u, next);
+                    __syncthreads();
+                }
+                return more;
+            }))
+            break;
 #pragma unroll
     for (int t = 0; t < NT; t++) {
         const uint32_t tok = t * 16u + r16;
         uint32_t orow = tok;
         if constexpr (ROUTED) orow = tok < live ? col[tok] : 0u;
 #pragma unroll
-        for (int m = 0; m < (int)kBkTiles; m++)
+        for (int m = 0; m < kTiles; m++)
 #pragma unroll
             for (int i = 0; i < 4; i++) {
-                const uint32_t row = c0 * 16u + (wave * kBkTiles + m) * 16u + g * 4u + i;
+                const uint32_t row = c0 * 16u + (wave * kTiles + m) * 16u + g * 4u + i;
                 if (tok < live && row < outDim) o[(size_t)orow * outDim + row] = acc[m][t][i];
             }
     }
 }
 
-template <int NT, int AUX, int VEC>
+template <int G, int NT, int LB>
 __global__ __launch_bounds__(kBkThreads) void bucket_gemm_rows_kernel(const uint16_t* __restrict__ B, uint32_t pitch, uint32_t cols,
                                                                       const uint16_t* __restrict__ xh, float* __restrict__ dst, uint32_t inDim,
-                                                                      uint32_t outDim, uint32_t rows, uint32_t per) {
-    extern __shared__ __attribute__((aligned(16))) unsigned char bk_lds[];
-    bucket_rows_body<NT, AUX, VEC, false>(bk_lds, B, pitch, cols, xh, dst + (size_t)blockIdx.y * rows * outDim, inDim, outDim, rows, rows, per, nullptr, 0u);
-}
-
-template <int AUX, int VEC>
+                                                                      uint32_t outDim, uint32_t rows, uint32_t per, uint32_t splits) {
+    extern __shared__ __attribute__((aligned(16))) unsigned char bk_lds_mem[];
+    uint32_t c0, split;
+    if (!bk_locate<G>(cols, splits, c0, split)) return;
+    bucket_rows_body<G, NT, LB, false>(bk_lds_mem, B, pitch, cols, xh, dst + (size_t)split * rows * outDim, inDim, outDim, rows, rows, per, nullptr, 0u, c0,
+                                            split);
+}
+
+template <int G, int LB>
 __global__ __launch_bounds__(kBkThreads) void bucket_gemm_rows_routed_kernel(const uint16_t* __restrict__ B, uint32_t pitch, uint32_t cols,
                                                                              const uint16_t* __restrict__ xh, float* __restrict__ dst,
                                                                              const uint32_t* __restrict__ cnt, const uint32_t* __restrict__ list,
                                                                              uint32_t inDim, uint32_t outDim, uint32_t assigns, uint32_t xRows,
-                                                                             uint32_t xShift, uint32_t per) {
-    extern __shared__ __attribute__((aligned(16))) unsigned char bk_lds[];
+                                                                             uint32_t xShift, uint32_t per, uint32_t splits) {
+    extern __shared__ __attribute__((aligned(16))) unsigned char bk_lds_mem[];
     __shared__ uint32_t col[64];
     const uint32_t e = blockIdx.z, n = __builtin_amdgcn_readfirstlane(min(cnt[e], kPfMaxAssign));
-    if (n == 0u) return;
+    uint32_t c0, split;
+    if (n == 0u || !bk_locate<G>(cols, splits, c0, split)) return;
     const uint16_t* Be = reinterpret_cast<const uint16_t*>(reinterpret_cast<const unsigned char*>(B) + (size_t)e * 16u * inDim * pitch);
-    float* o = dst + (size_t)blockIdx.y * assigns * outDim;
+    float* o = dst + (size_t)split * assigns * outDim;
     for (uint32_t a0 = 0; a0 < n; a0 += 64u) {
         const uint32_t live = min(n - a0, 64u);
         if (threadIdx.x < live) col[threadIdx.x] = min(list[e * kPfMaxAssign + a0 + threadIdx.x], assigns - 1u);
         __syncthreads();
         switch ((live + 15u) / 16u) {
-            case 1: bucket_rows_body<1, AUX, VEC, true>(bk_lds, Be, pitch, cols, xh, o, inDim, outDim, live, xRows, per, col, xShift); break;
-            case 2: bucket_rows_body<2, AUX, VEC, true>(bk_lds, Be, pitch, cols, xh, o, inDim, outDim, live, xRows, per, col, xShift); break;
-            case 3: bucket_rows_body<3, AUX, VEC, true>(bk_lds, Be, pitch, cols, xh, o, inDim, outDim, live, xRows, per, col, xShift); break;
-            default: bucket_rows_body<4, AUX, VEC, true>(bk_lds, Be, pitch, cols, xh, o, inDim, outDim, live, xRows, per, col, xShift); break;
+            case 1: bucket_rows_body<G, 1, LB, true>(bk_lds_mem, Be, pitch, cols, xh, o, inDim, outDim, live, xRows, per, col, xShift, c0, split); break;
+            case 2: bucket_rows_body<G, 2, LB, true>(bk_lds_mem, Be, pitch, cols, xh, o, inDim, outDim, live, xRows, per, col, xShift, c0, split); break;
+            case 3: bucket_rows_body<G, 3, LB, true>(bk_lds_mem, Be, pitch, cols, xh, o, inDim, outDim, live, xRows, per, col, xShift, c0, split); break;
+            default: bucket_rows_body<G, 4, LB, true>(bk_lds_mem, Be, pitch, cols, xh, o, inDim, outDim, live, xRows, per, col, xShift, c0, split); break;
         }
         __syncthreads();
     }
@@ -201,61 +251,68 @@
     return hipGetLastError();
 }
 
-static bool bucket_wide(const uint16_t* B, uint32_t pitch, uint32_t cols) {
-    return pitch % 16u == 0 && reinterpret_cast<uintptr_t>(B) % 16u == 0 && cols % 8u == 0;
-}
-
-template <int NT, int AUX, int VEC>
-static hipError_t launch_bucket_gemm_rows_t(const uint16_t* B, uint32_t pitch, uint32_t cols, const uint16_t* xh, float* dst, uint32_t inDim,
-                                            uint32_t outDim, uint32_t rows, PfSplit sp, hipStream_t st) {
-    const hipError_t e = allow_full_lds(reinterpret_cast<const void*>(&bucket_gemm_rows_kernel<NT, AUX, VEC>));
-    if (e != hipSuccess) return e;
-    hipLaunchKernelGGL((bucket_gemm_rows_kernel<NT, AUX, VEC>), dim3((cols + kBkCols - 1u) / kBkCols, sp.splits), dim3(kBkThreads), kBkLds, st,
-                       B, pitch, cols, xh, dst, inDim, outDim, rows, sp.per);
-    return hipGetLastError();
-}
-template <int NT>
-static hipError_t launch_bucket_gemm_rows_nt(bool nt, bool wide, const uint16_t* B, uint32_t pitch, uint32_t cols, const uint16_t* xh, float* dst,
-                                             uint32_t inDim, uint32_t outDim, uint32_t rows, PfSplit sp, hipStream_t st) {
-    if (nt) return wide ? launch_bucket_gemm_rows_t<NT, 2, 4>(B, pitch, cols, xh, dst, inDim, outDim, rows, sp, st)
-                        : launch_bucket_gemm_rows_t<NT, 2, 1>(B, pitch, cols, xh, dst, inDim, outDim, rows, sp, st);
-    return wide ? launch_bucket_gemm_rows_t<NT, 0, 4>(B, pitch, cols, xh, dst, inDim, outDim, rows, sp, st)
-                : launch_bucket_gemm_rows_t<NT, 0, 1>(B, pitch, cols, xh, dst, inDim, outDim, rows, sp, st);
+uint32_t bucket_group_cols(uint32_t inDim, uint32_t outDim, uint32_t numCU) {
+    const uint32_t cols = outDim / 16u, splits = pf_split(inDim, outDim).splits;
+    uint32_t best = 4u, bestCost = 0xFFFFFFFFu;
+    for (uint32_t G = 4u; G <= 32u; G *= 2u) {
+        const uint32_t wgs = (cols + G - 1u) / G * splits, cost = (G <= 8u ? 1u : G / 8u) * (wgs > numCU ? wgs : numCU);
+        if (cost < bestCost) { best = G; bestCost = cost; }
+    }
+    return best;
+}
+bool bucket_group_ok(uint32_t G) { return G == 4u || G == 8u || G == 16u || G == 32u; }
+
+struct BkChoice { uint32_t G; bool wide; };
+static BkChoice bk_choice(const uint16_t* B, uint32_t pitch, uint32_t inDim, uint32_t outDim, uint32_t numCU, uint32_t pinG) {
+    const uint32_t G = pinG ? pinG : bucket_group_cols(inDim, outDim, numCU), lb = G * 2u < 16u ? G * 2u : 16u;
+    return BkChoice{G, pitch % lb == 0 && reinterpret_cast<uintptr_t>(B) % lb == 0 && outDim / 16u % (lb / 2u) == 0};
+}
+template <class F>
+static hipError_t bk_with(const BkChoice& ch, F&& f) {
+    auto with_g = [&](auto G) {
+        constexpr int kWide = 2 * decltype(G)::value < 16 ? 2 * decltype(G)::value : 16;
+        return ch.wide ? f(G, std::integral_constant<int, kWide>{}) : f(G, std::integral_constant<int, 4>{});
+    };
+    switch (ch.G) {
+        case 4: return with_g(std::integral_constant<int, 4>{});
+        case 8: return with_g(std::integral_constant<int, 8>{});
+        case 16: return with_g(std::integral_constant<int, 16>{});
+        case 32: return with_g(std::integral_constant<int, 32>{});
+        default: return hipErrorInvalidValue;
+    }
 }
 
 hipError_t launch_bucket_gemm_rows(const uint16_t* B, uint32_t pitch, const float* x, uint16_t* xh, float* part, float* out, uint32_t inDim,
-                                   uint32_t outDim, uint32_t rows, hipStream_t st) {
+                                   uint32_t outDim, uint32_t rows, uint32_t numCU, uint32_t pinG, hipStream_t st) {
     if (rows < 1u || rows > (uint32_t)kPrefillMaxRows) return hipErrorInvalidValue;
     hipError_t e = launch_rows_to_f16(x, xh, rows * inDim, st);
     if (e != hipSuccess) return e;
     const PfSplit sp = pf_split(inDim, outDim);
     float* dst = sp.splits > 1u ? part : out;
     const uint32_t cols = outDim / 16u;
-    const bool nt = (size_t)inDim * outDim * 2u > kPfKeepBytes, wide = bucket_wide(B, pitch, cols);
-    switch ((rows + 15u) / 16u) {
-        case 1: e = launch_bucket_gemm_rows_nt<1>(nt, wide, B, pitch, cols, xh, dst, inDim, outDim, rows, sp, st); break;
-        case 2: e = launch_bucket_gemm_rows_nt<2>(nt, wide, B, pitch, cols, xh, dst, inDim, outDim, rows, sp, st); break;
-        case 3: e = launch_bucket_gemm_rows_nt<3>(nt, wide, B, pitch, cols, xh, dst, inDim, outDim, rows, sp, st); break;
-        default: e = launch_bucket_gemm_rows_nt<4>(nt, wide, B, pitch, cols, xh, dst, inDim, outDim, rows, sp, st); break;
-    }
+    e = bk_with(bk_choice(B, pitch, inDim, outDim, numCU, pinG), [&](auto G, auto LB) {
+        auto launch = [&](auto NT) {
+            auto* kernel = &bucket_gemm_rows_kernel<decltype(G)::value, decltype(NT)::value, decltype(LB)::value>;
+            const hipError_t err = allow_full_lds(reinterpret_cast<const void*>(kernel));
+            if (err != hipSuccess) return err;
+            hipLaunchKernelGGL(kernel, dim3(bk_grid(decltype(G)::value, cols, sp.splits)), dim3(kBkThreads), bk_lds(decltype(G)::value), st,
+                               B, pitch, cols, xh, dst, inDim, outDim, rows, sp.per, sp.splits);
+            return hipGetLastError();
+        };
+        switch ((rows + 15u) / 16u) {
+            case 1: return launch(std::integral_constant<int, 1>{});
+            case 2: return launch(std::integral_constant<int, 2>{});
+            case 3: return launch(std::integral_constant<int, 3>{});
+            default: return launch(std::integral_constant<int, 4>{});
+        }
+    });
     if (e != hipSuccess || sp.splits == 1u) return e;
     return launch_reduce_splits(part, out, rows * outDim, sp.splits, st);
 }
 
-template <int AUX, int VEC>
-static hipError_t launch_bucket_gemm_rows_routed_t(const uint16_t* B, uint32_t pitch, uint32_t cols, uint32_t numExperts, const uint16_t* xh, float* dst,
-                                                   const uint32_t* cnt, const uint32_t* list, uint32_t inDim, uint32_t outDim, uint32_t assigns,
-                                                   uint32_t xRows, uint32_t xShift, PfSplit sp, hipStream_t st) {
-    const hipError_t e = allow_full_lds(reinterpret_cast<const void*>(&bucket_gemm_rows_routed_kernel<AUX, VEC>));
-    if (e != hipSuccess) return e;
-    hipLaunchKernelGGL((bucket_gemm_rows_routed_kernel<AUX, VEC>), dim3((cols + kBkCols - 1u) / kBkCols, sp.splits, numExperts), dim3(kBkThreads), kBkLds, st,
-                       B, pitch, cols, xh, dst, cnt, list, inDim, outDim, assigns, xRows, xShift, sp.per);
-    return hipGetLastError();
-}
-
 hipError_t launch_bucket_gemm_rows_routed(const uint16_t* B, uint32_t pitch, uint32_t numExperts, const uint32_t* idx2, const float* x, uint32_t xPerSlot,
                                           uint16_t* xh, float* part, uint32_t* groups, float* out, uint32_t inDim, uint32_t outDim, uint32_t rows,
-                                          hipStream_t st) {
+                                          uint32_t numCU, uint32_t pinG, hipStream_t st) {
     if (rows < 1u || rows > (uint32_t)kPrefillMaxRows || numExperts < 1u || numExperts > kPfMaxExperts || xPerSlot > 1u) return hipErrorInvalidValue;
     const uint32_t assigns = 2u * rows, xRows = xPerSlot ? assigns : rows, cols = outDim / 16u;
     uint32_t* cnt = groups;
@@ -265,12 +322,14 @@
     const PfSplit sp = pf_split(inDim, outDim);
     float* dst = sp.splits > 1u ? part : out;
     const uint32_t xShift = xPerSlot ? 0u : 1u;
-    const bool nt = (size_t)inDim * outDim * 2u > kPfKeepBytes;
-    const bool wide = bucket_wide(B, pitch, cols);
-    if (nt) e = wide ? launch_bucket_gemm_rows_routed_t<2, 4>(B, pitch, cols, numExperts, xh, dst, cnt, list, inDim, outDim, assigns, xRows, xShift, sp, st)
-                     : launch_bucket_gemm_rows_routed_t<2, 1>(B, pitch, cols, numExperts, xh, dst, cnt, list, inDim, outDim, assigns, xRows, xShift, sp, st);
-    else e = wide ? launch_bucket_gemm_rows_routed_t<0, 4>(B, pitch, cols, numExperts, xh, dst, cnt, list, inDim, outDim, assigns, xRows, xShift, sp, st)
-                  : launch_bucket_gemm_rows_routed_t<0, 1>(B, pitch, cols, numExperts, xh, dst, cnt, list, inDim, outDim, assigns, xRows, xShift, sp, st);
+    e = bk_with(bk_choice(B, pitch, inDim, outDim, numCU, pinG), [&](auto G, auto LB) {
+        auto* kernel = &bucket_gemm_rows_routed_kernel<decltype(G)::value, decltype(LB)::value>;
+        const hipError_t err = allow_full_lds(reinterpret_cast<const void*>(kernel));
+        if (err != hipSuccess) return err;
+        hipLaunchKernelGGL(kernel, dim3(bk_grid(decltype(G)::value, cols, sp.splits), 1, numExperts), dim3(kBkThreads), bk_lds(decltype(G)::value), st,
+                           B, pitch, cols, xh, dst, cnt, list, inDim, outDim, assigns, xRows, xShift, sp.per, sp.splits);
+        return hipGetLastError();
+    });
     if (e != hipSuccess || sp.splits == 1u) return e;
     return launch_reduce_splits(part, out, assigns * outDim, sp.splits, st);
 }
diff --git a/include/effort_hip_debug.h b/include/effort_hip_debug.h
--- a/include/effort_hip_debug.h
+++ b/include/effort_hip_debug.h
@@ -34,6 +34,8 @@
 #define EFFORT_LANES_JOIN 2
 #define EFFORT_LANES_OUT_WORDS 18
 EFFORT_API int effort_debug_lanes(int lanes, int nOps, const int64_t* ops, int64_t nWords, int64_t* out);
+EFFORT_API int effort_debug_bucket_group(int inDim, int outDim, int numCU);
+EFFORT_API int effort_debug_set_bucket_group(effort_ctx* ctx, int cols);
 EFFORT_API int effort_debug_trace(effort_ctx* ctx, unsigned long long* host, int maxRecords);
 
 #ifdef __cplusplus
```

Result: slower. 21120 (-5.0%).
